# linchaobao/EPPM

Measured on AMD Instinct MI355X. Metric: Mflow-vectors/sec, higher is better.
Workload: dtype f32; 1 GPU; single 1024x436 Sintel-shape synthetic pair per step, full 3-level pyramid, patch_r=9, default defs.h parameters; 1 rank(s), independent pairs; inputs: RGBA planes resident in HBM before the timed region; outputs: interleaved float2 flow left in HBM (the PCIe-inclusive window of the reference API -- host RGB in, host u/v out -- is `host_boundary`, with --full); inputs=device-resident RGBA, outputs=device-resident float2 flow, pairs_in_flight_per_gpu=24, pairs_per_launch=8, contexts_in_flight=3, width=1024, height=436

## Files before the change

### eppm_amd/_lib.py

```python
import ctypes as C
import os

from .build import lib_path


class EppmError(RuntimeError):
    pass


class CParams(C.Structure):
    _fields_ = [("patch_r", C.c_int), ("num_iter", C.c_int), ("search_range", C.c_int), ("num_guess", C.c_int),
                ("seg_len", C.c_int), ("wmf_iters", C.c_int), ("seed", C.c_ulonglong), ("propagation", C.c_int),
                ("levels", C.c_int)]


class CTrackParams(C.Structure):
    _fields_ = [("spacing", C.c_int), ("min_eig", C.c_int64), ("fb_alpha", C.c_float), ("fb_beta", C.c_float), ("mb_alpha", C.c_float),
                ("mb_beta", C.c_float), ("capacity", C.c_int)]


class CTFilterParams(C.Structure):
    _fields_ = [("thresh", C.c_float), ("n_max", C.c_int)]


# ... 64 lines not shown


class CObject(C.Structure):
    _fields_ = [("id", C.c_int32), ("age", C.c_int32), ("area", C.c_int32), ("x0", C.c_int32), ("y0", C.c_int32), ("x1", C.c_int32),
                ("y1", C.c_int32), ("n_flow", C.c_int32), ("sum_x", C.c_int64), ("sum_y", C.c_int64), ("sum_qu", C.c_int64), ("sum_qv", C.c_int64)]

    def as_dict(self):
        return {k: int(getattr(self, k)) for k, _ in self._fields_}


class CObjectsCounts(C.Structure):
    _fields_ = [("n", C.c_int32), ("n_found", C.c_int32), ("n_components", C.c_int32), ("next_id", C.c_int32)]

    def as_dict(self):
        return {k: int(getattr(self, k)) for k, _ in self._fields_}


class CTrackCounts(C.Structure):
    _fields_ = [("live", C.c_int), ("ended", C.c_int), ("seeded", C.c_int), ("dropped", C.c_int), ("frame", C.c_int), ("next_id", C.c_int)]

    def as_dict(self):
        return {k: int(getattr(self, k)) for k, _ in self._fields_}


_lib = None

SYMBOLS = [
    "eppm_default_params", "eppm_create", "eppm_create_batch", "eppm_batch_size", "eppm_batch_set_images", "eppm_batch_set_images_device",
    "eppm_batch_compute", "eppm_batch_compute_device", "eppm_batch_compute_end", "eppm_batch_get_plane", "eppm_destroy", "eppm_set_stream", "eppm_set_images", "eppm_set_images_device",
    "eppm_compute", "eppm_compute_begin", "eppm_compute_end", "eppm_compute_device", "eppm_synchronize", "eppm_num_levels", "eppm_level_dims", "eppm_get_plane",
    "eppm_stage_times", "eppm_clear_stage_times", "eppm_enable_stage_timing", "eppm_last_error", "eppm_version",
    "eppm_device_count", "eppm_set_device", "eppm_malloc_device", "eppm_malloc_pitched", "eppm_free_device",
    "eppm_memcpy_h2d", "eppm_memcpy_d2h", "eppm_memcpy2d_h2d", "eppm_memcpy2d_d2h", "eppm_memset_device",
    "eppm_device_synchronize", "eppm_device_mem_info", "eppm_device_pci_bus_id", "eppm_bind_thread_to_device", "eppm_release_cached_memory", "eppm_set_launcher_stream", "eppm_set_launcher_params", "eppm_launcher_status",
    "baoCudaPatchMatchMultiscalePrepare", "baoCudaCensusTransform", "baoCudaPatchMatch", "baoCudaLeftRightCheck",
    "baoCudaOutlierRemoval", "baoCudaWeightedMedianFilter", "baoCudaFillHole", "baoCudaNNF2Flow", "baoCudaBLF_C2F",
    "baoCudaBLFCostFilterRefine", "baoCudaFlowSmoothing", "eppm_flow_to_color", "eppm_compute_color",
    "eppm_pm_rng_create", "eppm_pm_rng_reset", "eppm_pm_rng_destroy", "eppm_pm_rng_block_states", "eppm_pm_gen_rand_field",
    "eppm_pm_cost_field", "eppm_pm_seg_propagate", "eppm_pm_jump_propagate", "eppm_pm_parallel_propagate", "eppm_pm_random_search", "eppm_gauss_filter_rgba", "eppm_resize_rgba",
    "eppm_resize_flow",
    "eppm_host_register", "eppm_host_unregister", "eppm_host_is_registered", "eppm_host_alloc", "eppm_host_free",
    "eppm_compute_begin_into", "eppm_batch_compute_begin_into",
    "eppm_load_ppm", "eppm_ppm_size", "eppm_save_flo", "eppm_load_flo", "eppm_flo_size", "eppm_flow_error",
    "eppm_flow_error_border", "eppm_flow_error_percentage", "eppm_flow_cutoff", "eppm_flow_to_color_host",
    "eppm_compute_bidirectional", "eppm_compute_bidirectional_device", "eppm_batch_compute_bidirectional", "eppm_set_occlusion_params",
    "eppm_fb_occlusion", "eppm_fb_occlusion_host",
    "eppm_interpolate", "eppm_interpolate_device", "eppm_batch_interpolate", "eppm_interpolate_frames", "eppm_interpolate_host",
    "eppm_track_default_params", "eppm_track_capacity", "eppm_tracker_create", "eppm_tracker_destroy", "eppm_track_step",
    "eppm_track_step_frames", "eppm_tracker_get", "eppm_tracker_get_ended", "eppm_tracker_set", "eppm_track_step_host", "eppm_track_seeds_host",
    "eppm_push_image", "eppm_push_image_device", "eppm_set_temporal", "eppm_temporal_reset", "eppm_temporal_valid", "eppm_temporal_prior_host",
    "eppm_temporal_prior",
    "eppm_batch_set_temporal", "eppm_batch_push_images", "eppm_batch_push_images_device", "eppm_batch_temporal_valid", "eppm_batch_temporal_reset",
    "eppm_temporal_prior_batch",
    "eppm_set_stop_level", "eppm_stop_level", "eppm_flow_upsample",
    "eppm_tfilter_default_params", "eppm_tfilter_create", "eppm_tfilter_create_size", "eppm_tfilter_destroy", "eppm_tfilter_reset", "eppm_tfilter_step",
    "eppm_tfilter_step_frames", "eppm_tfilter_get", "eppm_tfilter_get_device", "eppm_tfilter_get_state", "eppm_tfilter_set_state",
    "eppm_tfilter_seed_host", "eppm_tfilter_step_host",
    "eppm_stab_default_params", "eppm_stab_create", "eppm_stab_create_size", "eppm_stab_destroy", "eppm_stab_reset", "eppm_stab_step",
    "eppm_stab_step_frames", "eppm_stab_get", "eppm_stab_get_device", "eppm_stab_get_mask", "eppm_stab_get_model", "eppm_stab_get_path",
    "eppm_stab_set_path", "eppm_gmotion_fit_host", "eppm_stab_update_host", "eppm_stab_warp_host",
    "eppm_cutdet_default_params", "eppm_cutdet_create", "eppm_cutdet_create_size", "eppm_cutdet_destroy", "eppm_cutdet_step",
    "eppm_cutdet_step_frames", "eppm_cutdet_get", "eppm_cutdet_cuts", "eppm_cutdet_host",
    "eppm_mblur_default_params", "eppm_motion_blur", "eppm_motion_blur_device", "eppm_batch_motion_blur", "eppm_motion_blur_frames",
    "eppm_motion_blur_host",
    "eppm_cmap_default_params", "eppm_cmap_create", "eppm_cmap_create_size", "eppm_cmap_destroy", "eppm_cmap_reset", "eppm_cmap_step",
    "eppm_cmap_step_frames", "eppm_cmap_get_state", "eppm_cmap_set_state", "eppm_cmap_set_layer", "eppm_cmap_render", "eppm_cmap_render_device",
    "eppm_cmap_age", "eppm_cmap_step_host", "eppm_cmap_render_host",
    "eppm_objects_default_params", "eppm_objects_create", "eppm_objects_create_size", "eppm_objects_destroy", "eppm_objects_reset",
    "eppm_objects_step", "eppm_objects_step_frames", "eppm_objects_get", "eppm_objects_get_labels", "eppm_objects_get_state",
    "eppm_objects_set_state", "eppm_objects_label_host", "eppm_objects_carry_host", "eppm_objects_assign_host",
    "eppm_plate_default_params", "eppm_plate_create", "eppm_plate_create_size", "eppm_plate_destroy", "eppm_plate_reset", "eppm_plate_canvas_dims",
    "eppm_plate_step", "eppm_plate_step_frames", "eppm_plate_render", "eppm_plate_render_frames", "eppm_plate_get", "eppm_plate_get_device",
    "eppm_plate_get_mask", "eppm_plate_get_path", "eppm_plate_set_path", "eppm_plate_get_state", "eppm_plate_set_state",
    "eppm_plate_forms_host", "eppm_plate_block_host", "eppm_plate_accumulate_host", "eppm_plate_render_host",
    "eppm_defect_default_params", "eppm_defect_create", "eppm_defect_create_size", "eppm_defect_destroy", "eppm_defect_reset", "eppm_defect_step",
    "eppm_defect_step_frames", "eppm_defect_get", "eppm_defect_get_device", "eppm_defect_get_mask", "eppm_defect_get_stats",
    "eppm_defect_get_state", "eppm_defect_set_state", "eppm_defect_step_host",
    "eppm_deflicker_default_params", "eppm_deflicker_create", "eppm_deflicker_create_size", "eppm_deflicker_destroy", "eppm_deflicker_reset",
    "eppm_deflicker_step", "eppm_deflicker_step_frames", "eppm_deflicker_get", "eppm_deflicker_get_device", "eppm_deflicker_get_field",
    "eppm_deflicker_get_stats", "eppm_deflicker_get_state", "eppm_deflicker_set_state", "eppm_deflicker_step_host",
]


TEST_SYMBOLS = ["eppm_test_set_option", "eppm_test_c2f_refine_batch", "eppm_test_c2f_refine_pre", "eppm_test_c2f_refine_probe", "eppm_probe_c2f_pretest", "eppm_probe_c2f_window", "eppm_probe_dispatch", "eppm_probe_fast_exp", "eppm_probe_div_const", "eppm_probe_delta_table",
                "eppm_probe_unpack_texel", "eppm_probe_pm_parity", "eppm_probe_ctx_rng_states", "eppm_test_pm_search", "eppm_probe_search_pretest", "eppm_probe_launch_log"]

_variant = None


def select_library(variant):
    global _variant
    if _lib is not None and variant != _variant:
        raise EppmError("select_library: a library is loaded already")
    _variant = variant


def lib():
    global _lib
    if _lib is None:
        path = lib_path(_variant)
        if not os.path.exists(path):
            raise EppmError(f"{path} is missing: run eppm_amd.build() (hipcc --offload-arch=gfx950); there is no CPU fallback")
        L = C.CDLL(path)
        L.eppm_last_error.restype = C.c_char_p
        L.eppm_version.restype = C.c_char_p
        _plate_signatures(L)
        _lib = L
    return _lib


def _plate_signatures(L):
    P, I, Z, F = C.c_void_p, C.c_int, C.c_size_t, C.c_float
    sig = {
        "eppm_plate_default_params": [P], "eppm_plate_create": [P, P, P], "eppm_plate_create_size": [I, I, I, I, P, P], "eppm_plate_destroy": [P],
        "eppm_plate_reset": [P, I], "eppm_plate_canvas_dims": [P, P, P], "eppm_plate_step": [P, P, P],
        "eppm_plate_step_frames": [P, I, P, Z, P, P, I], "eppm_plate_render": [P, P, I, P, Z, P],
        "eppm_plate_render_frames": [P, I, P, Z, P, P, P, Z, P], "eppm_plate_get": [P, I, P, Z, P], "eppm_plate_get_device": [P, I, P, Z],
        "eppm_plate_get_mask": [P, I, P], "eppm_plate_get_path": [P, I, P], "eppm_plate_set_path": [P, I, P], "eppm_plate_get_state": [P, I, P],
        "eppm_plate_set_state": [P, I, P], "eppm_plate_forms_host": [P, P, P, P], "eppm_plate_block_host": [P, P, I, I, P],
        "eppm_plate_accumulate_host": [P, P, P, P, I, I, P], "eppm_plate_render_host": [P, P, I, P, P, I, I, P, P, P],
    }
    for name, args in sig.items():
        fn = getattr(L, name, None)
        if fn is None:
            continue
        fn.argtypes = args
        fn.restype = I


def check(status, what=""):
    if status != 0:
        raise EppmError(f"{what}: status {status}: {lib().eppm_last_error().decode()}")


def check_launcher(what=""):
    check(lib().eppm_launcher_status(), what)


LAUNCH_STAGES = ("smoothing", "jbu", "refine", "search", "sweep", "sweeps_merged")


class launch_log:

    def __enter__(self):
        check(lib().eppm_test_set_option(b"launch_log", 1), "launch_log on")
        self._kept = None
        return self

    def entries(self):
        if self._kept is not None:
            return self._kept
        n = lib().eppm_probe_launch_log(None, 0)
        buf = (C.c_int * (6 * max(n, 1)))()
        n = min(n, lib().eppm_probe_launch_log(buf, n))
        return [(LAUNCH_STAGES[buf[6 * i]],) + tuple(buf[6 * i + 1:6 * i + 6]) for i in range(n)]

    def __exit__(self, *exc):
        self._kept = self.entries()
        lib().eppm_test_set_option(b"launch_log", 0)
        return False


def probe_dispatch(stage, *args, nout=1):
    a = (C.c_int * len(args))(*[int(v) for v in args])
    out = (C.c_int * nout)()
    check(lib().eppm_probe_dispatch(stage.encode(), a, len(args), out, nout), f"eppm_probe_dispatch {stage}")
    return tuple(out)
```

### eppm_amd/csrc/api_internal.h

```cpp
#pragma once

#include <ctype.h>
#include <math.h>
#include <sched.h>
#include <stdarg.h>
#include <stdio.h>
#include <stdlib.h>
#include <string.h>

#include <atomic>
#include <chrono>
#include <condition_variable>
#include <map>
#include <mutex>
#include <string>
#include <tuple>
#include <vector>

#include "eppm_internal.h"
#include "host_registry.h"

#define EPPM_HIDDEN __attribute__((visibility("hidden")))

EPPM_HIDDEN int set_err(int code, const char* fmt, ...) __attribute__((format(printf, 2, 3)));
#define HIPCHK(expr)                                                                                         \
    do {                                                                                                     \
        hipError_t e_ = (expr);                                                                              \
        if (e_ != hipSuccess) {                                                                              \
            (void)hipGetLastError();                                                                         \
            return set_err(EPPM_ERR_HIP, "%s failed: %s (%s:%d)", #expr, hipGetErrorString(e_), __FILE__, __LINE__); \
        }                                                                                                    \
    } while (0)
#define CHK(expr)                     \
    do {                              \
        int r_ = (expr);              \
        if (r_ != EPPM_OK) return r_; \
    } while (0)

EPPM_HIDDEN int check_params(const eppm_params& p);
EPPM_HIDDEN void host_pm_lut(int R, std::vector<float>& v);
EPPM_HIDDEN void host_wmf_lut(std::vector<float>& v);
EPPM_HIDDEN void host_blf_lut(std::vector<float>& v);
EPPM_HIDDEN int pyr_init_dim(int* arrH, int* arrW, int h, int w, int maxDepth, double ratio);
EPPM_HIDDEN int upload_lut(float** dst, const std::vector<float>& v);
struct DeltaIndex { int32_t t1[256]; std::vector<float> dval; };
EPPM_HIDDEN const DeltaIndex& delta_index();
EPPM_HIDDEN int upload_lut_delta(float** dst, const std::vector<float>& head, int which);
EPPM_HIDDEN int upload_pm_lut(float** dst, int R);
EPPM_HIDDEN int upload_wmf_lut(float** dst);
EPPM_HIDDEN int upload_blf_lut(float** dst);

#ifdef EPPM_TEST_HOOKS
EPPM_HIDDEN extern std::atomic<int> g_opt_rand_table;
EPPM_HIDDEN extern std::atomic<int> g_opt_sweep_spec;
EPPM_HIDDEN extern std::atomic<int> g_opt_no_split;
EPPM_HIDDEN extern std::atomic<int> g_opt_force_split;
EPPM_HIDDEN extern std::atomic<int> g_opt_search_pre;
static inline int opt_rand_table() { return g_opt_rand_table.load(); }
static inline int opt_sweep_spec() { return g_opt_sweep_spec.load(); }
static inline int opt_no_split() { return g_opt_no_split.load(); }
static inline int opt_force_split() { return g_opt_force_split.load(); }
static inline int opt_search_pre() { return g_opt_search_pre.load(); }
EPPM_HIDDEN extern std::atomic<int> g_opt_c2f_pre;
static inline int opt_c2f_pre() { return g_opt_c2f_pre.load(); }
EPPM_HIDDEN extern std::atomic<int> g_opt_alloc_fill;
static inline int opt_alloc_fill() { return g_opt_alloc_fill.load(); }
EPPM_HIDDEN hipError_t alloc_fill(hipError_t e, void* p, size_t bytes, bool pinned);
#else
static constexpr int opt_rand_table() { return 1; }
static constexpr int opt_sweep_spec() { return -1; }
static constexpr int opt_no_split() { return 0; }
static constexpr int opt_force_split() { return 0; }
static constexpr int opt_search_pre() { return -1; }
static constexpr int opt_c2f_pre() { return -1; }
static constexpr int opt_alloc_fill() { return -1; }
#endif


namespace eppm { struct RngTables; }
struct eppm_pm_rng {
    eppm::RngTables* tables = nullptr;
    const int16_t* rand_tab = nullptr;
    size_t rand_stride = 0;
    int device = 0, w = 0, h = 0, gx = 0, gy = 0, G = 0, per_lane = 0;
    unsigned long long seed = 0;
    uint32_t* init_tab = nullptr;
    uint32_t* iter_tab = nullptr;
    uint32_t* work[2][2] = {{nullptr, nullptr}, {nullptr, nullptr}};
    bool own_work = true;
    int cur[2] = {0, 0};
    uint32_t* skip_mat = nullptr;
    uint32_t skip_weyl = 0;
    eppm::PmRngDev dev() const
    {
        eppm::PmRngDev d;
        d.init_tab = init_tab; d.iter_tab = iter_tab; d.skip_mat = skip_mat;
        d.skip_weyl = skip_weyl; d.per_lane = per_lane; d.gx = gx; d.gy = gy;
        return d;
    }
};
EPPM_HIDDEN int rng_create(eppm_pm_rng** out, int w, int h, const eppm_params& p, bool alloc_work = true);
EPPM_HIDDEN void rng_free(eppm_pm_rng* r);
EPPM_HIDDEN void rngtab_release_idle();

EPPM_HIDDEN hipError_t cache_alloc(void** p, size_t bytes, bool pinned, int device);
EPPM_HIDDEN void cache_free(void* p, size_t bytes, bool pinned, int device);
EPPM_HIDDEN hipError_t pooled_stream_create(hipStream_t* out, int device);
EPPM_HIDDEN void pooled_stream_destroy(hipStream_t s, int device);

EPPM_HIDDEN eppm::PmProblem mk_problem(const eppm::PlanesH& P, float* cost, int16_t* nnf, int16_t* nnf_alt, eppm_pm_rng* rng, int k, float* spec = nullptr,
                                       int32_t* scand = nullptr, uint32_t* wl = nullptr, int16_t* seed = nullptr, float* restw = nullptr);
EPPM_HIDDEN void search(eppm::PmBatch& b, eppm_pm_rng* rng, const float* lut, const eppm_params& prm, hipStream_t s, int launch_no = -1, bool pretest = false);
EPPM_HIDDEN bool sweep_list_on(int mode);
EPPM_DECISION bool sweep_speculative(int iteration, long long pixels, int m);
EPPM_DECISION bool sweeps_merged(int iteration, long long pixels, long long problem_pixels, int m);
EPPM_HIDDEN void sweep(eppm::PmBatch& b, const float* lut, const eppm_params& prm, int dir, hipStream_t s, bool speculative = false);
EPPM_HIDDEN void jump(eppm::PmBatch& b, const float* lut, const eppm_params& prm, hipStream_t s);
EPPM_HIDDEN void neighbor(eppm::PmBatch& b, const float* lut, const eppm_params& prm, int launches, hipStream_t s);
EPPM_HIDDEN void run_patchmatch(eppm::PmBatch& b, eppm_pm_rng* rng, const float* lut, const eppm_params& prm, hipStream_t s, int spec_mode, int pre_from = -1);
EPPM_HIDDEN void pm_start(eppm::PmBatch& b, eppm_pm_rng* rng, const float* lut, const eppm_params& prm, hipStream_t s, int pre_from = -1);
EPPM_HIDDEN void pm_iterate(eppm::PmBatch& b, eppm_pm_rng* rng, const float* lut, const eppm_params& prm, hipStream_t s, int spec_mode, int pre_from = -1);
#ifndef EPPM_SWEEP_CACHE
#define EPPM_SWEEP_CACHE 1
#endif

EPPM_HIDDEN int launcher_finish();

EPPM_HIDDEN int ctx_device(const eppm_ctx* c, int* h, int* w);
EPPM_HIDDEN void ctx_stage_begin(eppm_ctx* c, const char* name);
EPPM_HIDDEN void ctx_stage_end(eppm_ctx* c);

EPPM_HIDDEN int stab_step_on(eppm_stab* f, eppm::StabArgs& in, int slot0, const uint8_t* cut, hipStream_t s, eppm_ctx* timing);
EPPM_HIDDEN const uint8_t* stab_mask_device(const eppm_stab* f, size_t* slot_stride);
EPPM_HIDDEN const char* stab_model_device(const eppm_stab* f, size_t* slot_stride);
```

### eppm_amd/csrc/c2f_device.cuh

```cuda
#pragma once
#include "eppm_device.cuh"

#ifndef EPPM_C2F_UNROLL
#define EPPM_C2F_UNROLL 2
#endif
#ifndef EPPM_C2F_WAVES
#define EPPM_C2F_WAVES 4
#endif
#ifndef EPPM_C2F_WAVES_MIN
#define EPPM_C2F_WAVES_MIN 2
#endif
#define EPPM_C2F_OCC __attribute__((amdgpu_waves_per_eu(EPPM_C2F_WAVES_MIN, EPPM_C2F_WAVES)))
#ifndef EPPM_C2F_WIN_H
#ifdef EPPM_TOL
#define EPPM_C2F_WIN_H 50
#else
#define EPPM_C2F_WIN_H 48
#endif
#endif
#ifndef EPPM_C2F_PASS2
#define EPPM_C2F_PASS2 1
#endif
#ifndef EPPM_C2F_WIN_WAVES
#define EPPM_C2F_WIN_WAVES 4
#endif
#ifndef EPPM_C2F_PRE
#define EPPM_C2F_PRE 1
#endif
#ifndef EPPM_C2F_PRE_ROWS
#define EPPM_C2F_PRE_ROWS 5
#endif
#ifndef EPPM_C2F_PRE_EPS
#define EPPM_C2F_PRE_EPS 0x1p-13f
#endif
#ifndef EPPM_C2F_PRE_PARTS
#define EPPM_C2F_PRE_PARTS 1
#endif
#define EPPM_C2F_PRE_DMIN 0x1p-60f
#define EPPM_C2F_PRE_RHSMIN 0x1p-100f
#ifndef EPPM_C2F_SPLIT_BELOW_WAVES
#define EPPM_C2F_SPLIT_BELOW_WAVES 1024
#endif
#ifndef EPPM_C2F_WINDOW
#define EPPM_C2F_WINDOW 1
#endif
#ifndef EPPM_C2F_WINDOW17
#define EPPM_C2F_WINDOW17 1
#endif
#ifdef EPPM_TOL
#define EPPM_C2F_LOG2 true
#else
#define EPPM_C2F_LOG2 false
#endif
#define EPPM_PRAGMA_(x) _Pragma(#x)
#define EPPM_UNROLL(n) EPPM_PRAGMA_(unroll n)

namespace eppm {

__device__ __forceinline__ Planes to_dev(const PlanesH& h, size_t pstride = 0, unsigned pair = 0)
{
    Planes p;
    p.pk1 = pair_ptr((const float4*)h.pk1, pstride, pair); p.pk2 = pair_ptr((const float4*)h.pk2, pstride, pair);
    p.w = h.w; p.h = h.h; p.pitch = h.pitch;
    return p;
}

__device__ __forceinline__ float4 stage_texel(const uint32_t* __restrict__ pc, const float4* __restrict__ pk, unsigned idx)
{
    if (pc) { const uint32_t w = pc[idx]; return make_texel(w, w >> 24); }
    return pk[idx];
}

__device__ __forceinline__ bool c2f_unknown(float fvx, float fvy) { return fvx > kUnknownFlowThresh || fvy > kUnknownFlowThresh; }
__device__ __forceinline__ int c2f_centre(float f, int x) { return (int)(int16_t)(f2short(f) + x); }
__device__ __forceinline__ void c2f_store_flow(float* flow, int idx, int fx, int fy)
{
    flow[idx * 2] = (float)fx;
    flow[idx * 2 + 1] = (float)fy;
}
__device__ __forceinline__ float c2f_min(float a, float b) { return (a < b) ? a : b; }
__device__ __forceinline__ float c2f_min4(float c1, float c2, float c3, float c4) { return c2f_min(c1, c2f_min(c2, c2f_min(c3, c4))); }
template <class F>
__device__ __forceinline__ void c2f_select_best(float* flow, int x, int y, int ccx, int ccy, int w, int h, F cost_of)
{
    int bx = ccx, by = ccy;
    float min_cost = 999999;
#pragma unroll
    for (int m = 0; m < 3; m++) {
        const int cx = (int)(int16_t)(ccx + m - 1);
        if (cx < 0 || cx >= w) continue;
#pragma unroll
        for (int n = 0; n < 3; n++) {
            const int cy = (int)(int16_t)(ccy + n - 1);
            if (cy < 0 || cy >= h) continue;
            const float cv = cost_of(m, n);
            if (cv < min_cost) { min_cost = cv; bx = cx; by = cy; }
        }
    }
    flow[(y * w + x) * 2] = (float)(bx - x);
    flow[(y * w + x) * 2 + 1] = (float)(by - y);
}

template <int SPLIT>
__device__ __forceinline__ bool c2f_tile_origin(const Planes& P, int& x0, int& y0, int& part)
{
    const int tiles_x = (P.w + kBlock - 1) / kBlock, tiles = tiles_x * ((P.h + kBlock - 1) / kBlock);
    const int per_xcd = (tiles + 7) / 8;
    const int slot = SPLIT ? (blockIdx.x >> 3) / SPLIT : (blockIdx.x >> 3);
    part = SPLIT ? (blockIdx.x >> 3) % SPLIT : -1;
    const int tile = (blockIdx.x & 7) * per_xcd + slot;
    if (slot >= per_xcd || tile >= tiles) return false;
    x0 = (tile % tiles_x) * kBlock; y0 = (tile / tiles_x) * kBlock;
    return true;
}

template <int R> struct C2fSrcTile { static constexpr int TWU = kBlock + 2 * R, TW = (TWU + 15) / 16 * 16; };
template <int R> struct C2fPreList {
    static constexpr int PADB = (C2fSrcTile<R>::TW - C2fSrcTile<R>::TWU) * 16, KROWS = PADB ? (256 * 8 + PADB - 1) / PADB : 0;
    static constexpr int CAP = PADB ? (C2fSrcTile<R>::TWU - KROWS) * (PADB / 2) : 0;
// ... 298 lines not shown
```

### eppm_amd/csrc/context.cpp

```cpp
#include "context.h"

using namespace eppm;

extern "C" int eppm_destroy(eppm_ctx* c)
{
    if (!c) return EPPM_OK;
    (void)hipSetDevice(c->device);
    if (c->stream) (void)hipStreamSynchronize(c->stream);
    c->out_hold.release();
    clear_events(c, c->ev);
    clear_events(c, c->ev_prep);
    for (hipEvent_t e : c->ev_pool) (void)hipEventDestroy(e);
    cache_free(c->slab, c->slab_bytes, false, c->device);
    if (c->h_color) (void)hipHostFree(c->h_color);
    for (int q = 0; q < 2; q++) {
        cache_free(c->h_rgb[q], c->h_rgb_bytes, true, c->device);
        if (c->ev_rgb[q]) (void)hipEventDestroy(c->ev_rgb[q]);
    }
    if (c->ev_h2d) (void)hipEventDestroy(c->ev_h2d);
    cache_free(c->h_flow, c->h_flow_bytes, true, c->device);
    cache_free(c->bwd, c->bwd_bytes, false, c->device);
    cache_free(c->h_bwd, c->h_bwd_bytes, true, c->device);
    cache_free(c->itp, c->itp_bytes, false, c->device);
    cache_free(c->h_itp, c->h_itp_bytes, true, c->device);
// ... 11 lines not shown
    struct Entry { int device, R; float *pm, *wmf, *blf; };
    static std::mutex mu;
    static std::vector<Entry> tab;
    std::lock_guard<std::mutex> lk(mu);
    for (const Entry& e : tab)
        if (e.device == device && e.R == R) { *pm = e.pm; *wmf = e.wmf; *blf = e.blf; return EPPM_OK; }
    Entry e{device, R, nullptr, nullptr, nullptr};
    CHK(upload_pm_lut(&e.pm, R));
    CHK(upload_wmf_lut(&e.wmf));
    CHK(upload_blf_lut(&e.blf));
    tab.push_back(e);
    *pm = e.pm; *wmf = e.wmf; *blf = e.blf;
    return EPPM_OK;
}

static int ctx_alloc(eppm_ctx* c)
{
    const int h = c->h, w = c->w;
    Carve cv;
    auto pitch_of = [](size_t row_bytes) { return (row_bytes + 255) & ~(size_t)255; };
    c->raw_pitch = pitch_of((size_t)w * 4);
    for (uint32_t** p : {&c->raw1, &c->raw2}) cv.plane(p, c->raw_pitch * h);
    for (int i = 0; i < c->nl; i++) {
        c->ipitch[i] = pitch_of((size_t)c->W[i] * 4);
        c->cpitch[i] = pitch_of((size_t)c->W[i]);
        const size_t n = (size_t)c->W[i] * c->H[i];
        for (uint32_t** p : {&c->img1[i], &c->img2[i], &c->tmpu[i]}) cv.plane(p, c->ipitch[i] * c->H[i]);
        for (void** p : {&c->pk1[i], &c->pk2[i]}) cv.plane(p, n * 16);
        for (uint32_t** p : {&c->pc1[i], &c->pc2[i]}) cv.plane(p, n * 4);
        for (uint8_t** p : {&c->cen1[i], &c->cen2[i]}) cv.plane(p, c->cpitch[i] * c->H[i]);
        for (float** p : {&c->flow[i], &c->flow_tmp[i]}) cv.plane(p, n * 8);
        if (i < c->nl - 1 && c2f_refine_wants_split(c->W[i], c->H[i], c->prm.patch_r, 1, c->opt_no_split != 0)) cv.plane(&c->c2f_cost9[i], n * 36 * 4);
    }
    const int L = c->nl - 1;
    const size_t n2 = (size_t)c->W[L] * c->H[L];
#ifndef EPPM_TOL
    if (c->prm.patch_r == 9)
#endif
    {
        c->pp_pad = (c->prm.patch_r + 2) & ~1;
        c->pp_pitch = parity_pitch(c->W[L], c->pp_pad);
        for (uint32_t** p : {&c->pp1, &c->pp2}) cv.plane(p, (size_t)2 * c->H[L] * c->pp_pitch * 4);
    }
    for (int16_t** p : {&c->nnf1, &c->nnf2, &c->nnf_tmp, &c->nnf_tmp2}) cv.plane(p, n2 * 4);
    for (float** p : {&c->cost1, &c->cost2}) cv.plane(p, n2 * 4);
    for (float** p : {&c->spec1, &c->spec2}) cv.plane(p, n2 * 4 * 4);
    if (pm_search_pretest_form(c->W[L], c->H[L], c->prm.patch_r, 2, c->npairs))
        for (float** p : {&c->restw1, &c->restw2}) cv.plane(p, n2 * 4);
    for (int32_t** p : {&c->scand1, &c->scand2}) cv.plane(p, n2 * 4 * 4);
    for (uint32_t** p : {&c->wl1, &c->wl2}) cv.plane(p, pm_worklist_words(c->W[L], c->H[L], c->prm.seg_len) * 4);
    for (int16_t** p : {&c->seed1, &c->seed2}) cv.plane(p, n2 * 4 * 4);
    cv.plane(&c->wmf_ws, wmf_workspace_words(c->W[L], c->H[L], c->prm.wmf_iters) * 4);
    cv.plane(&c->d_rgb, (size_t)h * w * 3 * 2);
    cv.plane(&c->d_color, (size_t)h * w * 4);
    cv.plane(&c->d_uv, (size_t)h * w * 8);
    CHK(rng_create(&c->rng, c->W[L], c->H[L], c->prm, false));
    const size_t rng_bytes = (size_t)c->rng->gx * c->rng->gy * 64 * 6 * 4;
    for (int k = 0; k < 2; k++)
        for (int q = 0; q < 2; q++) cv.plane(&c->rng->work[k][q], rng_bytes);
    c->stride = (cv.off + 4095) & ~(size_t)4095;
    CHK(cv.alloc(&c->slab, &c->slab_bytes, c->stride * c->npairs, c->device, (std::to_string(c->npairs) + " slab(s)").c_str()));
    CHK(shared_luts(c->device, c->prm.patch_r, &c->lut_pm, &c->lut_wmf, &c->lut_blf));
    c->out_u.assign(c->npairs, nullptr);
    c->out_v.assign(c->npairs, nullptr);
    for (auto* v : {&c->tmp_snap, &c->tmp_valid, &c->tmp_seeded, &c->tmp_cut}) v->assign(c->npairs, 0);
    return EPPM_OK;
}

extern "C" int eppm_create_batch(eppm_ctx** out, int h, int w, int device, const eppm_params* params, int npairs)
{
    if (!out) return set_err(EPPM_ERR_ARG, "eppm_create: NULL out");
    *out = nullptr;
    if (npairs < 1 || npairs > 4096) return set_err(EPPM_ERR_ARG, "eppm_create_batch: npairs %d out of range [1,4096]", npairs);
    if (h < 4 || w < 4 || h > 32767 || w > 32767) return set_err(EPPM_ERR_ARG, "eppm_create: size %dx%d out of range (NNF coordinates are int16)", w, h);
    if ((unsigned long long)h * (unsigned long long)w * 16ULL >= (1ULL << 32))
        return set_err(EPPM_ERR_ARG, "eppm_create: size %dx%d out of range (texel planes are addressed with 32-bit byte offsets)", w, h);
    eppm_params p;
    eppm_default_params(&p);
    if (params) p = *params;
    CHK(check_params(p));
    HIPCHK(hipSetDevice(device));
    eppm_ctx* c = new eppm_ctx();
    c->device = device; c->prm = p; c->h = h; c->w = w; c->npairs = npairs; c->n_active = 1;
    c->opt_sweep_spec = opt_sweep_spec(); c->opt_no_split = opt_no_split(); c->opt_search_pre = opt_search_pre(); c->opt_c2f_pre = opt_c2f_pre();
    c->nl = pyr_init_dim(c->H, c->W, h, w, p.levels, 0.5f);
    const int L = c->nl - 1;
    if (c->H[L] < 1 || c->W[L] < 1 || (c->W[L] + p.seg_len - 1) / p.seg_len > 1024 || (c->H[L] + p.seg_len - 1) / p.seg_len > 1024) {
        delete c;
        return set_err(EPPM_ERR_ARG, "eppm_create: unsupported size %dx%d", w, h);
    }
    const hipError_t e = pooled_stream_create(&c->stream, c->device);
    if (e != hipSuccess) { delete c; return set_err(EPPM_ERR_HIP, "hipStreamCreate: %s", hipGetErrorString(e)); }
    c->own_stream = true;
    int r = ctx_alloc(c);
    if (r != EPPM_OK) { eppm_destroy(c); return r; }
    *out = c;
    return EPPM_OK;
}

extern "C" int eppm_create(eppm_ctx** out, int h, int w, int device, const eppm_params* params)
{
    return eppm_create_batch(out, h, w, device, params, 1);
}

extern "C" int eppm_batch_size(const eppm_ctx* c) { return c ? c->npairs : 0; }

extern "C" int eppm_set_stream(eppm_ctx* c, void* s)
{
    if (!c) return set_err(EPPM_ERR_ARG, "NULL ctx");
    if (c->own_stream && c->stream) { (void)hipStreamSynchronize(c->stream); pooled_stream_destroy(c->stream, c->device); }
    c->stream = (hipStream_t)s;
    c->own_stream = false;
    return EPPM_OK;
}

extern "C" int eppm_num_levels(const eppm_ctx* c) { return c ? c->nl : 0; }
extern "C" int eppm_level_dims(const eppm_ctx* c, int level, int* h, int* w)
{
    if (!c || level < 0 || level >= c->nl) return set_err(EPPM_ERR_ARG, "bad level");
    if (h) *h = c->H[level];
    if (w) *w = c->W[level];
    return EPPM_OK;
}
extern "C" int eppm_enable_stage_timing(eppm_ctx* c, int on)
{
    if (!c) return set_err(EPPM_ERR_ARG, "NULL ctx");
    c->timing = (on == 2) ? 2 : (on != 0);
    return EPPM_OK;
}

int ctx_device(const eppm_ctx* c, int* h, int* w)
{
    *h = c->h;
    *w = c->w;
    return c->device;
}

void ctx_stage_begin(eppm_ctx* c, const char* name) { stage_begin(c, c->ev, name); }
void ctx_stage_end(eppm_ctx* c) { stage_end(c, c->ev); }

extern "C" int eppm_synchronize(eppm_ctx* c)
{
    if (!c) return set_err(EPPM_ERR_ARG, "NULL ctx");
    HIPCHK(hipStreamSynchronize(c->stream));
    return EPPM_OK;
}

extern "C" int eppm_stage_times(eppm_ctx* c, const char** names, float* ms, int max)
{
    if (!c) return 0;
    (void)hipStreamSynchronize(c->stream);
    int n = 0;
    for (auto* v : {&c->ev_prep, &c->ev})
        for (auto& e : *v) {
            if (n >= max) return n;
            float t = 0;
            if (hipEventElapsedTime(&t, e.a, e.b) != hipSuccess) t = -1;
            names[n] = e.name; ms[n] = t; n++;
        }
    return n;
}

extern "C" int eppm_clear_stage_times(eppm_ctx* c)
{
    if (!c) return set_err(EPPM_ERR_ARG, "NULL ctx");
    (void)hipStreamSynchronize(c->stream);
    clear_events(c, c->ev);
// ... 86 lines not shown
```

### eppm_amd/csrc/context.h

```cpp
#pragma once

#include <algorithm>

#include "api_internal.h"

struct StageEv { const char* name; hipEvent_t a, b; };

struct eppm_ctx {
    int device = 0;
    hipStream_t stream = nullptr;
    bool own_stream = false;
    int opt_sweep_spec = -1, opt_no_split = 0, opt_search_pre = -1, opt_c2f_pre = -1;
    eppm_params prm;
    int h = 0, w = 0, nl = 0;
    int stop_level = 0;
    int npairs = 1, n_active = 1;
    char* slab = nullptr;
    size_t stride = 0;
    int H[eppm::kMaxLevels], W[eppm::kMaxLevels];
    size_t ipitch[eppm::kMaxLevels], cpitch[eppm::kMaxLevels];
    uint32_t *raw1 = nullptr, *raw2 = nullptr;
    size_t raw_pitch = 0;
    uint32_t *img1[eppm::kMaxLevels] = {}, *img2[eppm::kMaxLevels] = {}, *tmpu[eppm::kMaxLevels] = {};
    uint8_t *cen1[eppm::kMaxLevels] = {}, *cen2[eppm::kMaxLevels] = {};
    void *pk1[eppm::kMaxLevels] = {}, *pk2[eppm::kMaxLevels] = {};
    uint32_t *pc1[eppm::kMaxLevels] = {}, *pc2[eppm::kMaxLevels] = {};
    uint32_t *pp1 = nullptr, *pp2 = nullptr;
    int pp_pitch = 0, pp_pad = 0;
    int16_t *nnf1 = nullptr, *nnf2 = nullptr, *nnf_tmp = nullptr, *nnf_tmp2 = nullptr;
    float *cost1 = nullptr, *cost2 = nullptr;
    float *spec1 = nullptr, *spec2 = nullptr;
    int32_t *scand1 = nullptr, *scand2 = nullptr;
    uint32_t *wl1 = nullptr, *wl2 = nullptr;
    float *restw1 = nullptr, *restw2 = nullptr;
    int16_t *seed1 = nullptr, *seed2 = nullptr;
    uint32_t* wmf_ws = nullptr;
    bool flow_pending = false;
    float *flow[eppm::kMaxLevels] = {}, *flow_tmp[eppm::kMaxLevels] = {};
    float* c2f_cost9[eppm::kMaxLevels] = {};
    float *lut_pm = nullptr, *lut_wmf = nullptr, *lut_blf = nullptr;
    eppm_pm_rng* rng = nullptr;
    float* d_uv = nullptr;
    uint32_t* d_color = nullptr;
    uint32_t* h_color = nullptr;
    uint8_t* d_rgb = nullptr;
    size_t slab_bytes = 0, h_rgb_bytes = 0, h_flow_bytes = 0;
    uint8_t* h_rgb[2] = {nullptr, nullptr};
    hipEvent_t ev_rgb[2] = {nullptr, nullptr};
    hipEvent_t ev_h2d = nullptr;
    int rgb_cur = 0;
    float* h_flow = nullptr;
    std::vector<float*> out_u, out_v;
    eppm::HostHold out_hold;
    bool have_images = false, have_flow = false;
    char* bwd = nullptr;
    size_t bwd_stride = 0, bwd_bytes = 0, h_bwd_bytes = 0;
    float* bflow[eppm::kMaxLevels] = {};
    float* d_buv = nullptr;
    uint8_t *occ1 = nullptr, *occ2 = nullptr;
    uint8_t* h_bwd = nullptr;
    float occ_alpha = 0.01f, occ_beta = 0.5f;
    bool have_bwd = false;
    bool bwd_images = false;
    char* itp = nullptr;
    size_t itp_bytes = 0, itp_plane = 0, h_itp_bytes = 0;
    uint64_t* itp_keys = nullptr;
    int32_t *itp_fill1 = nullptr, *itp_fill2 = nullptr;
    uint8_t* itp_rgb = nullptr;
    uint8_t* h_itp = nullptr;
    char* mbl = nullptr;
    size_t mbl_bytes = 0, mbl_plane = 0, mbl_tplane = 0, h_mbl_bytes = 0;
    uint32_t* mbl_packed = nullptr;
    uint64_t* mbl_tkeys = nullptr;
    uint8_t* mbl_rgb = nullptr;
    uint8_t* h_mbl = nullptr;
    bool temporal = false;
    std::vector<uint8_t> tmp_snap;
    std::vector<uint8_t> tmp_valid;
    std::vector<uint8_t> tmp_seeded;
    std::vector<uint8_t> tmp_cut;
    char* tmp = nullptr;
    size_t tmp_bytes = 0, tmp_stride = 0;
    int16_t *prev_fwd = nullptr, *prev_bwd = nullptr, *prior1 = nullptr, *prior2 = nullptr, *nnf_init1 = nullptr, *nnf_init2 = nullptr;
    float *cost_init1 = nullptr, *cost_init2 = nullptr;
    int32_t* tmp_keys = nullptr;
    void tmp_drop() { std::fill(tmp_valid.begin(), tmp_valid.end(), 0); std::fill(tmp_snap.begin(), tmp_snap.end(), 0); std::fill(tmp_cut.begin(), tmp_cut.end(), 0); }
    int timing = 0;
    std::vector<StageEv> ev;
    std::vector<StageEv> ev_prep;
    std::vector<hipEvent_t> ev_pool;
    eppm::Batch bt() const { return eppm::Batch{n_active, stride}; }
    template <class T> T* of_pair(T* p, int k) const { return (T*)((char*)p + (size_t)k * stride); }
    template <class T> T* of_bwd_pair(T* p, int k) const { return (T*)((char*)p + (size_t)k * bwd_stride); }
};

static inline eppm::PlanesH planes(const eppm_ctx* c, int l, bool swap)
{
    eppm::PlanesH p;
    p.pk1 = swap ? c->pk2[l] : c->pk1[l];
    p.pk2 = swap ? c->pk1[l] : c->pk2[l];
    p.w = c->W[l]; p.h = c->H[l];
    p.pitch = c->W[l];
    p.pc1 = swap ? c->pc2[l] : c->pc1[l];
    p.pc2 = swap ? c->pc1[l] : c->pc2[l];
    if (l == c->nl - 1 && c->pp1) {
        p.pp1 = swap ? c->pp2 : c->pp1;
        p.pp2 = swap ? c->pp1 : c->pp2;
        p.pp_pitch = c->pp_pitch; p.pp_pad = c->pp_pad;
    }
    return p;
}

static inline hipEvent_t pool_event(eppm_ctx* c)
{
    hipEvent_t e = nullptr;
    if (!c->ev_pool.empty()) { e = c->ev_pool.back(); c->ev_pool.pop_back(); }
    else (void)hipEventCreate(&e);
    return e;
}
static inline bool stage_on(const eppm_ctx* c, bool dominant) { return c->timing == 1 || (c->timing == 2 && dominant); }
static inline void stage_begin(eppm_ctx* c, std::vector<StageEv>& v, const char* name, bool dominant = false)
{
    if (!stage_on(c, dominant)) return;
    StageEv e;
    e.name = name;
    e.a = pool_event(c);
    e.b = pool_event(c);
    (void)hipEventRecord(e.a, c->stream);
    v.push_back(e);
}
static inline void stage_end(eppm_ctx* c, std::vector<StageEv>& v, bool dominant = false)
{
    if (!stage_on(c, dominant)) return;
    (void)hipEventRecord(v.back().b, c->stream);
// ... 44 lines not shown
```

### eppm_amd/csrc/ctx_compute.cpp

```cpp
#include "context.h"
#include "temporal.h"

using namespace eppm;

static int tmp_alloc(eppm_ctx* c)
{
    if (c->tmp) return EPPM_OK;
    const int L = c->nl - 1;
    const size_t n2 = (size_t)c->W[L] * c->H[L];
    Carve cv;
    for (int16_t** p : {&c->prev_fwd, &c->prev_bwd, &c->prior1, &c->prior2, &c->nnf_init1, &c->nnf_init2}) cv.plane(p, n2 * 4);
    for (float** p : {&c->cost_init1, &c->cost_init2}) cv.plane(p, n2 * 4);
    cv.plane(&c->tmp_keys, n2 * 4 * 2);
    c->tmp_stride = cv.off;
    CHK(cv.alloc(&c->tmp, &c->tmp_bytes, c->tmp_stride * c->npairs, c->device, "temporal planes"));
    for (int k = 0; k < c->npairs; k++) launch_temporal_keys_init((int32_t*)((char*)c->tmp_keys + (size_t)k * c->tmp_stride), (int)(2 * n2), c->stream);
    HIPCHK(hipGetLastError());
    return EPPM_OK;
}

static int set_temporal(eppm_ctx* c, int on)
{
    c->temporal = on != 0;
    if (!on) c->tmp_drop();
    return EPPM_OK;
}
extern "C" int eppm_set_temporal(eppm_ctx* c, int on)
{
    if (!c) return set_err(EPPM_ERR_ARG, "eppm_set_temporal: NULL ctx");
    if (on && c->npairs != 1) return set_err(EPPM_ERR_ARG, "eppm_set_temporal: a batch context streams through eppm_batch_set_temporal (one clip per slot)");
    return set_temporal(c, on);
}
extern "C" int eppm_temporal_reset(eppm_ctx* c)
{
    if (!c) return set_err(EPPM_ERR_ARG, "eppm_temporal_reset: NULL ctx");
    return eppm_batch_temporal_reset(c, 0);
}
extern "C" int eppm_temporal_valid(const eppm_ctx* c) { return eppm_batch_temporal_valid(c, 0); }

extern "C" int eppm_batch_set_temporal(eppm_ctx* c, int on)
{
    if (!c) return set_err(EPPM_ERR_ARG, "eppm_batch_set_temporal: NULL ctx");
    return set_temporal(c, on);
}
extern "C" int eppm_batch_temporal_reset(eppm_ctx* c, int pair)
{
    if (!c) return set_err(EPPM_ERR_ARG, "eppm_batch_temporal_reset: NULL ctx");
    if (pair >= c->npairs) return set_err(EPPM_ERR_ARG, "eppm_batch_temporal_reset: pair %d, context holds %d", pair, c->npairs);
    for (int k = pair < 0 ? 0 : pair; k < (pair < 0 ? c->npairs : pair + 1); k++) c->tmp_valid[k] = c->tmp_snap[k] = 0;
    return EPPM_OK;
}
extern "C" int eppm_batch_temporal_valid(const eppm_ctx* c, int pair)
{
    return c && pair >= 0 && pair < c->npairs && c->temporal && c->tmp_valid[pair] ? 1 : 0;
}

struct Branch {
    int16_t *&nnf, *&nnf_alt;
    float* cost;
    uint32_t* const* guide;
    bool swap, bwd, dominant;
    int16_t* snapshot;
    float *a[kMaxLevels], *b[kMaxLevels];
};

enum { kStageUp, kStageRefine, kStageBlf, kStageJbu };
static const struct EPPM_HIDDEN LevelStageNames {
    char s[4][2][kMaxLevels][24];
    LevelStageNames()
    {
        const char* base[4] = {"upsample", "c2f_refine", "flow_blf", "flow_jbu"};
        for (int k = 0; k < 4; k++)
            for (int b = 0; b < 2; b++)
                for (int l = 0; l < kMaxLevels; l++) snprintf(s[k][b][l], sizeof s[k][b][l], "%s%s_L%d", base[k], b ? "_bwd" : "", l);
    }
} level_stage;

static void branch_nnf2flow(eppm_ctx* c, Branch& d)
{
    hipStream_t s = c->stream;
    const Batch bt = c->bt();
    const int L = c->nl - 1, lw = c->W[L], lh = c->H[L], gp = (int)(c->ipitch[L] / 4);
    launch_outlier(d.nnf_alt, d.cost, d.nnf, lw, lh, lw, lw, s, bt);
    std::swap(d.nnf, d.nnf_alt);
    if (launch_wmf(d.nnf, d.nnf_alt, d.guide[L], gp, lw, lh, lw, c->lut_wmf, c->prm.wmf_iters, 1, c->wmf_ws, s, bt) != d.nnf)
        std::swap(d.nnf, d.nnf_alt);
    launch_fill_holes(d.nnf_alt, d.nnf, d.guide[L], gp, lw, lh, lw, s, bt);
    std::swap(d.nnf, d.nnf_alt);
    if (d.snapshot) launch_nnf2flow_snapshot(d.a[L], lw, d.snapshot, c->tmp_stride, d.nnf, lw, lw, lh, s, bt);
    else launch_nnf2flow(d.a[L], lw, d.nnf, lw, lw, lh, s, bt);
}

static int branch_c2f(eppm_ctx* c, Branch& d, int (*keep)(eppm_ctx*, int, float*))
{
    hipStream_t s = c->stream;
    const Batch bt = c->bt();
    const int L = c->nl - 1;
    auto blf = [&](float* dst, const float* src, int l) { launch_flow_blf(dst, src, d.guide[l], (int)(c->ipitch[l] / 4), c->W[l], c->H[l], c->W[l], c->lut_blf, s, bt); };
    const int stop = c->stop_level;
    float* r = d.a[L];
    for (int l = L - 1; l >= 0; l--) {
        if (l < stop) {
            stage_begin(c, c->ev, level_stage.s[kStageJbu][d.bwd][l]);
            float* out = (r == d.b[l]) ? d.a[l] : d.b[l];
            launch_flow_jbu(out, r, d.guide[l], (int)(c->ipitch[l] / 4), c->W[l], c->H[l], c->W[l + 1], c->H[l + 1], c->lut_blf, s, bt);
            r = out;
            CHK(keep(c, l, r));
            stage_end(c, c->ev);
            continue;
        }
        stage_begin(c, c->ev, level_stage.s[kStageUp][d.bwd][l]);
        launch_resize_flow(d.a[l], c->H[l], c->W[l], r, c->H[l + 1], c->W[l + 1], 2.0f, 2.0f, s, bt);
        stage_end(c, c->ev);
        stage_begin(c, c->ev, level_stage.s[kStageRefine][d.bwd][l], d.dominant);
        launch_c2f_refine(planes(c, l, d.swap), d.a[l], c->lut_pm, c->prm.patch_r, c->c2f_cost9[l], s, bt, c->opt_no_split != 0, c->opt_c2f_pre);
        stage_end(c, c->ev, d.dominant);
        stage_begin(c, c->ev, level_stage.s[kStageBlf][d.bwd][l]);
        blf(d.b[l], d.a[l], l);
        r = d.b[l];
        if (l > 0) CHK(keep(c, l, r));
        stage_end(c, c->ev);
    }
    if (stop > 0) return EPPM_OK;
    stage_begin(c, c->ev, d.bwd ? "flow_blf_bwd_final" : "flow_blf_final");
    float* out = (r == d.b[0]) ? d.a[0] : d.b[0];
    blf(out, r, 0);
    CHK(keep(c, 0, out));
    stage_end(c, c->ev);
    return EPPM_OK;
}

static int keep_fwd(eppm_ctx* c, int l, float* r)
{
    if (r != c->flow[l]) std::swap(c->flow[l], c->flow_tmp[l]);
    return EPPM_OK;
}

static int compute_all(eppm_ctx* c)
{
    if (!c->have_images) return set_err(EPPM_ERR_STATE, "eppm_compute: no images set");
    HIPCHK(hipSetDevice(c->device));
    c->have_bwd = false;
    hipStream_t s = c->stream;
    const Batch bt = c->bt();
    const int L = c->nl - 1, lw = c->W[L], lh = c->H[L];

    const bool tmode = c->temporal;
    bool seeded = false;
    std::fill(c->tmp_seeded.begin(), c->tmp_seeded.end(), 0);
    if (tmode) {
        CHK(tmp_alloc(c));
        TemporalArgs a{};
        for (int k = 0; k < bt.n; k++)
            if (c->tmp_valid[k]) { a.armed[k >> 5] |= 1u << (k & 31); seeded = true; }
        if (seeded) {
            a.prev[0] = c->prev_fwd; a.prior[0] = c->prior1; a.keys[0] = c->tmp_keys; a.step[0] = 1;
            a.prev[1] = c->prev_bwd; a.prior[1] = c->prior2; a.keys[1] = c->tmp_keys + (size_t)lw * lh; a.step[1] = -1;
            a.w = lw; a.h = lh; a.ndir = 2; a.nslots = bt.n; a.stride = c->tmp_stride;
            stage_begin(c, c->ev, "temporal_advect");
            launch_temporal_splat(a, s);
            launch_temporal_gather(a, s);
            stage_end(c, c->ev);
        }
    }
    std::fill(c->tmp_snap.begin(), c->tmp_snap.end(), 0);

    const size_t pm_entry = c->ev.size();
    stage_begin(c, c->ev, "patchmatch");
    {
        PmBatch b;
        b.n = 2; b.cpitch = lw; b.npitch = lw; b.npairs = bt.n; b.stride = bt.stride;
        b.cache_plane = (size_t)lw * lh;
        b.seed_plane = (size_t)lw * lh * 2;
        b.wl_units = pm_worklist_units(lw, lh, c->prm.seg_len);
        b.p[0] = mk_problem(planes(c, L, false), c->cost1, c->nnf1, c->nnf_tmp, c->rng, 0, c->spec1, EPPM_SWEEP_CACHE ? c->scand1 : nullptr, sweep_list_on(c->opt_sweep_spec) ? c->wl1 : nullptr, c->seed1, c->restw1);
        b.p[1] = mk_problem(planes(c, L, true), c->cost2, c->nnf2, c->nnf_tmp2, c->rng, 1, c->spec2, EPPM_SWEEP_CACHE ? c->scand2 : nullptr, sweep_list_on(c->opt_sweep_spec) ? c->wl2 : nullptr, c->seed2, c->restw2);
        if (!seeded) run_patchmatch(b, c->rng, c->lut_pm, c->prm, s, c->opt_sweep_spec, c->opt_search_pre);
        else {
            pm_start(b, c->rng, c->lut_pm, c->prm, s, c->opt_search_pre);
            PmSeed sd;
            sd.prior[0] = c->prior1; sd.nnf_init[0] = c->nnf_init1; sd.cost_init[0] = c->cost_init1;
            sd.prior[1] = c->prior2; sd.nnf_init[1] = c->nnf_init2; sd.cost_init[1] = c->cost_init2;
            sd.stride = c->tmp_stride;
            stage_begin(c, c->ev, "temporal_select");
            launch_pm_cost_select(b, sd, c->lut_pm, c->prm.patch_r, s);
            stage_end(c, c->ev);
            pm_iterate(b, c->rng, c->lut_pm, c->prm, s, c->opt_sweep_spec, c->opt_search_pre);
        }
    }
    stage_end_at(c, c->ev, pm_entry);
    if (tmode) launch_temporal_snapshot(c->prev_bwd, c->tmp_stride, c->nnf2, lw, lw, lh, s, bt);

    stage_begin(c, c->ev, "l2_post");
    launch_lr_check(c->nnf1, c->cost1, c->nnf2, lw, lh, lw, lw, s, bt);
    launch_lr_check(c->nnf2, c->cost2, c->nnf1, lw, lh, lw, lw, s, bt);
    Branch d{c->nnf1, c->nnf_tmp, c->cost1, c->img1, false, false, true, tmode ? c->prev_fwd : nullptr};
    for (int l = 0; l <= L; l++) { d.a[l] = c->flow[l]; d.b[l] = c->flow_tmp[l]; }
    branch_nnf2flow(c, d);
    stage_end(c, c->ev);
    CHK(branch_c2f(c, d, keep_fwd));
    HIPCHK(hipGetLastError());
    c->have_flow = true;
    for (int k = 0; k < bt.n; k++) {
        c->tmp_snap[k] = tmode && !c->tmp_cut[k];
        c->tmp_seeded[k] = tmode && c->tmp_valid[k];
    }
    std::fill(c->tmp_valid.begin(), c->tmp_valid.end(), 0);
    return EPPM_OK;
}


static int bwd_alloc(eppm_ctx* c)
{
    if (c->bwd) return EPPM_OK;
    Carve cv;
    for (int l = 0; l < c->nl; l++) cv.plane(&c->bflow[l], (size_t)c->W[l] * c->H[l] * 8);
    const size_t n = (size_t)c->h * c->w;
    cv.plane(&c->d_buv, n * 10);
    c->bwd_stride = (cv.off + 4095) & ~(size_t)4095;
    CHK(cv.alloc(&c->bwd, &c->bwd_bytes, c->bwd_stride * c->npairs, c->device, "backward planes"));
    c->occ1 = (uint8_t*)c->d_buv + n * 8;
    c->occ2 = c->occ1 + n;
    return EPPM_OK;
}

static int keep_bwd(eppm_ctx* c, int l, float* src)
{
    const size_t bytes = (size_t)c->W[l] * c->H[l] * 8;
    for (int k = 0; k < c->n_active; k++)
        HIPCHK(hipMemcpyAsync(c->of_bwd_pair(c->bflow[l], k), c->of_pair(src, k), bytes, hipMemcpyDeviceToDevice, c->stream));
    return EPPM_OK;
}

static int backward_all(eppm_ctx* c)
{
    const int L = c->nl - 1;
    Branch d{c->nnf2, c->nnf_tmp2, c->cost2, c->img2, true, true, false, nullptr};
    for (int l = 0; l <= L; l++) { d.a[l] = c->flow_tmp[l]; d.b[l] = c->d_uv; }
    stage_begin(c, c->ev, "l2_post_bwd");
    branch_nnf2flow(c, d);
    if (L > 0) CHK(keep_bwd(c, L, d.a[L]));
    stage_end(c, c->ev);
    CHK(branch_c2f(c, d, keep_bwd));

    stage_begin(c, c->ev, "fb_occlusion");
    launch_fb_occlusion(c->occ1, c->occ2, c->flow[0], c->stride, c->bflow[0], c->bwd_stride, c->h, c->w, c->occ_alpha, c->occ_beta, c->n_active, 2, c->stream);
    stage_end(c, c->ev);
    HIPCHK(hipGetLastError());
    c->have_bwd = true;
    c->bwd_images = true;
    return EPPM_OK;
}

static int compute_bidir_all(eppm_ctx* c)
{
    if (!c->have_images) return set_err(EPPM_ERR_STATE, "eppm_compute_bidirectional: no images set");
    HIPCHK(hipSetDevice(c->device));
    CHK(bwd_alloc(c));
    CHK(compute_all(c));
    return backward_all(c);
}

extern "C" int eppm_compute_device(eppm_ctx* c, void* d_flow)
{
    if (!c) return set_err(EPPM_ERR_ARG, "NULL ctx");
    CHK(compute_all(c));
    if (d_flow) HIPCHK(hipMemcpyAsync(d_flow, c->flow[0], (size_t)c->h * c->w * 8, hipMemcpyDeviceToDevice, c->stream));
    return EPPM_OK;
}

extern "C" int eppm_batch_compute_device(eppm_ctx* c, void* const* d_flows)
{
    if (!c) return set_err(EPPM_ERR_ARG, "NULL ctx");
    CHK(compute_all(c));
    if (d_flows)
        for (int k = 0; k < c->n_active; k++)
            if (d_flows[k]) HIPCHK(hipMemcpyAsync(d_flows[k], c->of_pair(c->flow[0], k), (size_t)c->h * c->w * 8, hipMemcpyDeviceToDevice, c->stream));
    return EPPM_OK;
}

static int compute_begin_impl(eppm_ctx* c, int n_out, float* const* u, float* const* v, bool bidir)
{
    CHK(bidir ? compute_bidir_all(c) : compute_all(c));
    const size_t n = (size_t)c->h * c->w;
    launch_split_flow(c->d_uv, c->flow[0], (int)n, c->stream, c->bt());
    if (bidir) {
        launch_split_flow(c->d_buv, c->bflow[0], (int)n, c->stream, Batch{c->n_active, c->bwd_stride});
        HIPCHK(pinned_lazy(&c->h_bwd, &c->h_bwd_bytes, n * 10 * c->npairs, c->device));
        for (int k = 0; k < c->n_active; k++)
            HIPCHK(hipMemcpyAsync(c->h_bwd + (size_t)k * n * 10, c->of_bwd_pair(c->d_buv, k), n * 10, hipMemcpyDeviceToHost, c->stream));
    }
    for (int k = 0; k < c->n_active; k++) {
        float* du = (u && k < n_out) ? u[k] : nullptr;
        float* dv = (v && k < n_out) ? v[k] : nullptr;
        const float* src = c->of_pair(c->d_uv, k);
        if (du && dv && c->out_hold.add2(du, dv, n * 4)) {
            HIPCHK(hipMemcpyAsync(du, src, n * 4, hipMemcpyDeviceToHost, c->stream));
            HIPCHK(hipMemcpyAsync(dv, src + n, n * 4, hipMemcpyDeviceToHost, c->stream));
            c->out_u[k] = du; c->out_v[k] = dv;
            continue;
        }
        HIPCHK(pinned_lazy(&c->h_flow, &c->h_flow_bytes, n * 8 * c->npairs, c->device));
        HIPCHK(hipMemcpyAsync(c->h_flow + (size_t)k * n * 2, src, n * 8, hipMemcpyDeviceToHost, c->stream));
        c->out_u[k] = c->out_v[k] = nullptr;
    }
    c->flow_pending = true;
    return EPPM_OK;
}
static int compute_begin(eppm_ctx* c, int n_out, float* const* u, float* const* v, bool bidir = false)
{
    const int r = compute_begin_impl(c, n_out, u, v, bidir);
    if (r != EPPM_OK && !c->out_hold.v.empty()) {
        (void)hipStreamSynchronize(c->stream);
        c->out_hold.release();
    }
    return r;
}

extern "C" int eppm_compute_begin(eppm_ctx* c)
{
    if (!c) return set_err(EPPM_ERR_ARG, "eppm_compute_begin: NULL ctx");
    return compute_begin(c, 0, nullptr, nullptr);
}

extern "C" int eppm_compute_begin_into(eppm_ctx* c, float* u, float* v)
{
    if (!c || !u || !v) return set_err(EPPM_ERR_ARG, "eppm_compute_begin_into: NULL argument");
    return compute_begin(c, 1, &u, &v);
}

extern "C" int eppm_batch_compute_begin_into(eppm_ctx* c, float* const* u, float* const* v)
{
    if (!c || !u || !v) return set_err(EPPM_ERR_ARG, "eppm_batch_compute_begin_into: NULL argument");
    return compute_begin(c, c->n_active, u, v);
}

static int compute_end(eppm_ctx* c, int n_out, float* const* u, float* const* v)
{
    if (!c->flow_pending) return set_err(EPPM_ERR_STATE, "eppm_compute_end without eppm_compute_begin");
    HIPCHK(hipSetDevice(c->device));
    const hipError_t es = hipStreamSynchronize(c->stream);
    c->out_hold.release();
    HIPCHK(es);
    c->flow_pending = false;
    const size_t n = (size_t)c->h * c->w;
    for (int k = 0; k < n_out && k < c->n_active; k++) {
        if (!u[k] || !v[k]) continue;
        const float* fu = c->out_u[k] ? c->out_u[k] : c->h_flow + (size_t)k * n * 2;
        const float* fv = c->out_v[k] ? c->out_v[k] : c->h_flow + (size_t)k * n * 2 + n;
        if (u[k] != fu) memcpy(u[k], fu, n * sizeof(float));
        if (v[k] != fv) memcpy(v[k], fv, n * sizeof(float));
    }
    return EPPM_OK;
}

extern "C" int eppm_compute_end(eppm_ctx* c, float* u, float* v)
{
    if (!c || !u || !v) return set_err(EPPM_ERR_ARG, "eppm_compute_end: NULL argument");
    return compute_end(c, 1, &u, &v);
}

// ... 88 lines not shown
```

### eppm_amd/csrc/ctx_images.cpp

```cpp
#include "context.h"

using namespace eppm;

static int prepare(eppm_ctx* c, bool only2 = false)
{
    stage_begin(c, c->ev_prep, "prepare");
    hipStream_t s = c->stream;
    const Batch bt = c->bt();
    uint32_t **p1 = c->img1, **p2 = c->img2, **tmp = c->tmpu;
    const int p0 = (int)(c->ipitch[0] / 4);
    if (only2) launch_gauss_rgba(p2[0], c->raw2, p0, c->H[0], c->W[0], .5f, 2, s, bt);
    else launch_gauss_rgba2(p1[0], c->raw1, p2[0], c->raw2, p0, c->H[0], c->W[0], .5f, 2, s, bt);
    const float ratio = 0.5f;
    const float baseSigma = (1 / ratio - 1);
    const int n = (int)(log(0.25) / (double)logf(ratio));
    const float nSigma = baseSigma * n;
    for (int i = 1; i < c->nl; i++) {
        const int j = (i <= n) ? 0 : i - n;
        const float sigma = (i <= n) ? baseSigma * i : nSigma;
        const float r = (i <= n) ? (float)pow(ratio, i) : (float)pow(ratio, i) * c->W[0] / c->W[j];
        const int radius = (int)(sigma * 3);
        const int pj = (int)(c->ipitch[j] / 4), pi = (int)(c->ipitch[i] / 4);
        if (gauss_decimate2_ok(c->H[i], c->W[i], c->H[j], c->W[j], r, radius)) {
            if (only2) launch_gauss_decimate2(p2[i], p2[j], p2[i], p2[j], 1, pi, c->H[i], c->W[i], pj, c->H[j], c->W[j], sigma, radius, s, bt);
            else launch_gauss_decimate2(p1[i], p1[j], p2[i], p2[j], 2, pi, c->H[i], c->W[i], pj, c->H[j], c->W[j], sigma, radius, s, bt);
        } else {
            for (int k = only2 ? 1 : 0; k < 2; k++) {
                uint32_t** pyr = k ? p2 : p1;
                launch_gauss_rgba(tmp[j], pyr[j], pj, c->H[j], c->W[j], sigma, radius, s, bt);
                launch_resize_rgba(pyr[i], pi, c->H[i], c->W[i], tmp[j], pj, c->H[j], c->W[j], r, s, bt);
            }
        }
    }
    CensusBatch cb;
    cb.n = 0;
    for (int k = only2 ? 1 : 0; k < 2; k++)
        for (int i = 0; i < c->nl; i++) {
            CensusJob& J = cb.job[cb.n++];
            J.census = k ? c->cen2[i] : c->cen1[i]; J.cpitch = (int)c->cpitch[i];
            J.texels = k ? c->pk2[i] : c->pk1[i];   J.tpitch = c->W[i];
            J.img = k ? c->img2[i] : c->img1[i];    J.ipitch = (int)(c->ipitch[i] / 4);
            J.w = c->W[i]; J.h = c->H[i]; J.first_block = 0;
            J.packed = k ? c->pc2[i] : c->pc1[i];
        }
    launch_census_batch(cb, s, bt);
    if (c->pp1) {
        const int L = c->nl - 1;
        if (!only2) launch_parity_planes(c->pp1, c->pp_pitch, c->pp_pad, c->pc1[L], c->W[L], c->W[L], c->H[L], s, bt);
        launch_parity_planes(c->pp2, c->pp_pitch, c->pp_pad, c->pc2[L], c->W[L], c->W[L], c->H[L], s, bt);
    }
    stage_end(c, c->ev_prep);
    HIPCHK(hipGetLastError());
    c->have_images = true;
    c->have_flow = false;
    c->bwd_images = false;
    return EPPM_OK;
}

static int upload_rgb(eppm_ctx* c, uint8_t* dst, const uint8_t* src, size_t row_stride, HostHold& hold, int slot, bool* direct, bool* staged)
{
    const size_t row = (size_t)c->w * 3, img = row * c->h, span = row_stride * (c->h - 1) + row;
    if (hold.add(src, span)) {
        if (row_stride == row) HIPCHK(hipMemcpyAsync(dst, src, img, hipMemcpyHostToDevice, c->stream));
        else HIPCHK(hipMemcpy2DAsync(dst, row, src, row_stride, row, c->h, hipMemcpyHostToDevice, c->stream));
        *direct = true;
        return EPPM_OK;
    }
    const int q = c->rgb_cur;
    if (!*staged) {
        HIPCHK(pinned_lazy(&c->h_rgb[q], &c->h_rgb_bytes, img * 2 * c->npairs, c->device));
        if (!c->ev_rgb[q]) HIPCHK(hipEventCreateWithFlags(&c->ev_rgb[q], hipEventDisableTiming));
        else HIPCHK(hipEventSynchronize(c->ev_rgb[q]));
    }
    uint8_t* h = c->h_rgb[q] + (size_t)slot * img;
    copy_rows(h, row, src, row_stride, row, c->h);
    HIPCHK(hipMemcpyAsync(dst, h, img, hipMemcpyHostToDevice, c->stream));
    *staged = true;
    return EPPM_OK;
}
static int upload_done(eppm_ctx* c, bool direct, bool staged)
{
    if (staged) {
        HIPCHK(hipEventRecord(c->ev_rgb[c->rgb_cur], c->stream));
        c->rgb_cur ^= 1;
    }
    if (direct) {
        if (!c->ev_h2d) HIPCHK(hipEventCreateWithFlags(&c->ev_h2d, hipEventDisableTiming));
        HIPCHK(hipEventRecord(c->ev_h2d, c->stream));
    }
    return EPPM_OK;
}

static int set_images_host_impl(eppm_ctx* c, int n, const uint8_t* const* rgb1, const uint8_t* const* rgb2, size_t row_stride, HostHold& hold)
{
    if (row_stride < (size_t)c->w * 3) return set_err(EPPM_ERR_ARG, "eppm_set_images: row_stride %zu < 3*w", row_stride);
    HIPCHK(hipSetDevice(c->device));
    const size_t img = (size_t)c->w * 3 * c->h;
    for (int k = 0; k < n; k++)
        if (!rgb1[k] || !rgb2[k]) return set_err(EPPM_ERR_ARG, "eppm_set_images: NULL image");
    bool staged = false, direct = false;
    for (int k = 0; k < n; k++)
        for (int f = 0; f < 2; f++)
            CHK(upload_rgb(c, c->of_pair(c->d_rgb, k) + (size_t)f * img, f ? rgb2[k] : rgb1[k], row_stride, hold, k * 2 + f, &direct, &staged));
    CHK(upload_done(c, direct, staged));
    c->n_active = n;
    c->tmp_drop();
    const int p0 = (int)(c->raw_pitch / 4);
    launch_rgb_to_rgba(c->raw1, p0, c->d_rgb, c->h, c->w, c->stream, c->bt());
    launch_rgb_to_rgba(c->raw2, p0, c->d_rgb + img, c->h, c->w, c->stream, c->bt());
    const int r = prepare(c);
    if (direct) HIPCHK(hipEventSynchronize(c->ev_h2d));
    return r;
}
static int set_images_host(eppm_ctx* c, int n, const uint8_t* const* rgb1, const uint8_t* const* rgb2, size_t row_stride)
{
    HostHold hold;
    const int r = set_images_host_impl(c, n, rgb1, rgb2, row_stride, hold);
    if (r != EPPM_OK && !hold.v.empty()) (void)hipStreamSynchronize(c->stream);
    return r;
}

extern "C" int eppm_set_images(eppm_ctx* c, const uint8_t* rgb1, const uint8_t* rgb2, size_t row_stride)
{
    if (!c || !rgb1 || !rgb2) return set_err(EPPM_ERR_ARG, "eppm_set_images: NULL argument");
    return set_images_host(c, 1, &rgb1, &rgb2, row_stride);
}

extern "C" int eppm_batch_set_images(eppm_ctx* c, int n, const uint8_t* const* rgb1, const uint8_t* const* rgb2, size_t row_stride)
{
    if (!c || !rgb1 || !rgb2) return set_err(EPPM_ERR_ARG, "eppm_batch_set_images: NULL argument");
    if (n < 1 || n > c->npairs) return set_err(EPPM_ERR_ARG, "eppm_batch_set_images: %d pairs, context holds %d", n, c->npairs);
    return set_images_host(c, n, rgb1, rgb2, row_stride);
}

static int set_images_device(eppm_ctx* c, int n, const void* const* d1, const void* const* d2, size_t pitch)
{
    if (pitch < (size_t)c->w * 4 || (pitch & 3)) return set_err(EPPM_ERR_ARG, "eppm_set_images_device: bad pitch %zu", pitch);
    HIPCHK(hipSetDevice(c->device));
    for (int k = 0; k < n; k++) {
        if (!d1[k] || !d2[k]) return set_err(EPPM_ERR_ARG, "eppm_set_images_device: NULL image");
        HIPCHK(hipMemcpy2DAsync(c->of_pair(c->raw1, k), c->raw_pitch, d1[k], pitch, (size_t)c->w * 4, c->h, hipMemcpyDeviceToDevice, c->stream));
        HIPCHK(hipMemcpy2DAsync(c->of_pair(c->raw2, k), c->raw_pitch, d2[k], pitch, (size_t)c->w * 4, c->h, hipMemcpyDeviceToDevice, c->stream));
    }
    c->n_active = n;
    c->tmp_drop();
    return prepare(c);
}

extern "C" int eppm_set_images_device(eppm_ctx* c, const void* d1, const void* d2, size_t pitch)
{
    if (!c || !d1 || !d2) return set_err(EPPM_ERR_ARG, "eppm_set_images_device: NULL argument");
    return set_images_device(c, 1, &d1, &d2, pitch);
}

extern "C" int eppm_batch_set_images_device(eppm_ctx* c, int n, const void* const* d_rgba1, const void* const* d_rgba2, size_t pitch)
{
    if (!c || !d_rgba1 || !d_rgba2) return set_err(EPPM_ERR_ARG, "eppm_batch_set_images_device: NULL argument");
    if (n < 1 || n > c->npairs) return set_err(EPPM_ERR_ARG, "eppm_batch_set_images_device: %d pairs, context holds %d", n, c->npairs);
    return set_images_device(c, n, d_rgba1, d_rgba2, pitch);
}

static int push_check(eppm_ctx* c, const char* what, bool batch = false)
{
    if (!batch && c->npairs != 1) return set_err(EPPM_ERR_ARG, "%s: a batch context takes one frame per slot (eppm_batch_push_images)", what);
    if (!c->have_images) return set_err(EPPM_ERR_STATE, "%s: no pair set yet (eppm_set_images first)", what);
    if (c->flow_pending) return set_err(EPPM_ERR_STATE, "%s: an eppm_compute_begin is pending", what);
    return EPPM_OK;
}
static void push_swap(eppm_ctx* c, const uint8_t* new_clip = nullptr)
{
    for (int k = 0; k < c->n_active; k++) {
        const bool cut = new_clip && new_clip[k];
        c->tmp_valid[k] = c->temporal && c->tmp_snap[k] && !cut;
        c->tmp_snap[k] = 0;
        c->tmp_cut[k] = cut;
    }
    std::swap(c->raw1, c->raw2);
    for (int l = 0; l < c->nl; l++) {
        std::swap(c->img1[l], c->img2[l]);
        std::swap(c->cen1[l], c->cen2[l]);
        std::swap(c->pk1[l], c->pk2[l]);
        std::swap(c->pc1[l], c->pc2[l]);
    }
    std::swap(c->pp1, c->pp2);
}

static int push_image_host_impl(eppm_ctx* c, const uint8_t* rgb, size_t row_stride, HostHold& hold)
{
    if (row_stride < (size_t)c->w * 3) return set_err(EPPM_ERR_ARG, "eppm_push_image: row_stride %zu < 3*w", row_stride);
    HIPCHK(hipSetDevice(c->device));
    uint8_t* dst = c->d_rgb + (size_t)c->w * 3 * c->h;
    bool staged = false, direct = false;
    CHK(upload_rgb(c, dst, rgb, row_stride, hold, 1, &direct, &staged));
    CHK(upload_done(c, direct, staged));
    push_swap(c);
    launch_rgb_to_rgba(c->raw2, (int)(c->raw_pitch / 4), dst, c->h, c->w, c->stream, c->bt());
    const int r = prepare(c, true);
    if (direct) HIPCHK(hipEventSynchronize(c->ev_h2d));
    return r;
}

extern "C" int eppm_push_image(eppm_ctx* c, const uint8_t* rgb, size_t row_stride)
{
    if (!c || !rgb) return set_err(EPPM_ERR_ARG, "eppm_push_image: NULL argument");
    CHK(push_check(c, "eppm_push_image"));
    HostHold hold;
    const int r = push_image_host_impl(c, rgb, row_stride, hold);
    if (r != EPPM_OK && !hold.v.empty()) (void)hipStreamSynchronize(c->stream);
    return r;
}

extern "C" int eppm_push_image_device(eppm_ctx* c, const void* d_rgba, size_t pitch)
{
    if (!c || !d_rgba) return set_err(EPPM_ERR_ARG, "eppm_push_image_device: NULL argument");
    CHK(push_check(c, "eppm_push_image_device"));
    if (pitch < (size_t)c->w * 4 || (pitch & 3)) return set_err(EPPM_ERR_ARG, "eppm_push_image_device: bad pitch %zu", pitch);
    HIPCHK(hipSetDevice(c->device));
    HIPCHK(hipMemcpy2DAsync(c->raw1, c->raw_pitch, d_rgba, pitch, (size_t)c->w * 4, c->h, hipMemcpyDeviceToDevice, c->stream));
    push_swap(c);
    return prepare(c, true);
}

static int push_images_host_impl(eppm_ctx* c, int n, const uint8_t* const* rgb, size_t row_stride, const uint8_t* new_clip, HostHold& hold)
{
    if (row_stride < (size_t)c->w * 3) return set_err(EPPM_ERR_ARG, "eppm_batch_push_images: row_stride %zu < 3*w", row_stride);
    for (int k = 0; k < n; k++)
        if (!rgb[k]) return set_err(EPPM_ERR_ARG, "eppm_batch_push_images: NULL image");
    HIPCHK(hipSetDevice(c->device));
    const size_t img = (size_t)c->w * 3 * c->h;
// ... 36 lines not shown
```

### eppm_amd/csrc/eppm_internal.h

```cpp
#pragma once

#include <hip/hip_runtime.h>
#include <stddef.h>
#include <stdint.h>

#include <atomic>

#include "../../include/eppm.h"

namespace eppm {

constexpr int kMaxLevels = 8;
constexpr int kNumLevels = 3;
constexpr int kBlock = 16;
constexpr int kMaxS = 32;
constexpr int kWmfRadius = 4;
constexpr int kBlfRadius = 10;
constexpr int kDeltaSlots = 800;

struct Batch {
    int n;
    size_t stride;
};
constexpr Batch kOnePair = {1, 0};

#define EPPM_DECISION __attribute__((visibility("hidden")))
enum LaunchStage { kLaunchSmoothing = 0, kLaunchJbu, kLaunchRefine, kLaunchSearch, kLaunchSweep, kLaunchSweepsMerged };
typedef void (*LaunchNoteFn)(int stage, int w, int h, int npairs, int form, int extra);
extern EPPM_DECISION std::atomic<LaunchNoteFn> g_launch_note;
inline void launch_note(int stage, int w, int h, int npairs, int form, int extra = 0)
{
    if (LaunchNoteFn f = g_launch_note.load(std::memory_order_relaxed)) f(stage, w, h, npairs, form, extra);
}

struct PlanesH {
    const void* pk1;
    const void* pk2;
    int w, h, pitch;
    const uint32_t* pc1 = nullptr;
    const uint32_t* pc2 = nullptr;
    const uint32_t* pp1 = nullptr;
    const uint32_t* pp2 = nullptr;
    int pp_pitch = 0, pp_pad = 0;
};
inline int parity_pitch(int w, int pad) { return (w + 2 * pad + 1) / 2 + 1; }
void launch_parity_planes(uint32_t* pp, int pp_pitch, int pad, const uint32_t* pc, int pc_pitch, int w, int h, hipStream_t s, Batch bt = kOnePair);

void launch_gauss_rgba(uint32_t* out, const uint32_t* in, int pitch_px, int h, int w, float sigma, int radius, hipStream_t s, Batch bt = kOnePair);
bool gauss_decimate2_ok(int outH, int outW, int h, int w, float ratio, int radius);
void launch_gauss_decimate2(uint32_t* out0, const uint32_t* in0, uint32_t* out1, const uint32_t* in1, int nimg, int out_pitch_px, int outH,
                            int outW, int pitch_px, int h, int w, float sigma, int radius, hipStream_t s, Batch bt = kOnePair);
void launch_gauss_rgba2(uint32_t* out0, const uint32_t* in0, uint32_t* out1, const uint32_t* in1, int pitch_px, int h, int w, float sigma,
                        int radius, hipStream_t s, Batch bt = kOnePair);
struct CensusJob { uint8_t* census; int cpitch; void* texels; int tpitch; const uint32_t* img; int ipitch; int w, h; int first_block;
                   uint32_t* packed = nullptr; };
struct CensusBatch { int n; CensusJob job[2 * kMaxLevels]; };
void launch_census_batch(CensusBatch& B, hipStream_t s, Batch bt = kOnePair);
void launch_resize_rgba(uint32_t* out, int out_pitch_px, int outH, int outW, const uint32_t* in, int in_pitch_px, int h, int w,
                        float ratio, hipStream_t s, Batch bt = kOnePair);
void launch_census(uint8_t* census, int cpitch, void* texels, int tpitch, const uint32_t* img, int ipitch, int w, int h, hipStream_t s);
void launch_pack(void* texels, int tpitch, const uint32_t* img, int ipitch, const uint8_t* census, int cpitch, int w, int h, hipStream_t s);
void launch_delta_values(float* t2, int n, int which, hipStream_t s);
void launch_rgb_to_rgba(uint32_t* out, int pitch_px, const uint8_t* rgb, int h, int w, hipStream_t s, Batch bt = kOnePair);

struct PmProblem {
    PlanesH P;
    float* cost;
    int16_t* nnf;
    int16_t* nnf_alt;
    float* spec = nullptr;
    int32_t* scand = nullptr;
    uint32_t* wl = nullptr;
    int16_t* seed = nullptr;
    uint32_t* rng_work;
    uint32_t* rng_work_next;
    float* restw = nullptr;
};
struct PmBatch {
    PmProblem p[2];
    int n;
    int cpitch, npitch;
    int npairs = 1;
    size_t stride = 0;
    size_t cache_plane = 0;
    int wl_units = 0;
    int sweep_seq = 0;
    size_t seed_plane = 0;
    int merged_it = 0;
    int seg_len = 0, nseg_row = 0, nseg_col = 0;
};
int pm_worklist_units(int w, int h, int seg_len);
inline size_t pm_worklist_words(int w, int h, int seg_len) { return 16 + 10 * (size_t)pm_worklist_units(w, h, seg_len); }
struct PmRngDev {
    const uint32_t* init_tab;
    const uint32_t* iter_tab;
    const uint32_t* skip_mat;
    uint32_t skip_weyl;
    int per_lane;
    int gx, gy;
    const int16_t* rand_tab = nullptr;
};
void launch_pm_rand_table(const PmRngDev& rng, uint32_t* work, int16_t* tab, int G, hipStream_t s);
void launch_pm_init_field(const PmBatch& b, const PmRngDev& rng, hipStream_t s);
void launch_pm_cost_field(const PmBatch& b, const float* lut, int R, hipStream_t s);
int pm_parity_kernels(int R);
bool launch_pm_sweep(PmBatch& b, const float* lut, int R, int seg_len, int dir, hipStream_t s, bool speculative = false);
bool launch_pm_sweeps_merged(PmBatch& b, const float* lut, int R, int seg_len, int iteration, hipStream_t s);
void launch_pm_jump(const PmBatch& b, const float* lut, int R, int step, hipStream_t s);
void launch_pm_neighbor(const PmBatch& b, const float* lut, int R, hipStream_t s);
void launch_pm_random_search(const PmBatch& b, const PmRngDev& rng, const float* lut, int R, int search_range, int num_guess,
                             hipStream_t s, bool pretest = false);
void launch_pm_rest_weight(const PmBatch& b, const float* lut, int R, hipStream_t s);
bool pm_search_pretest_ready(const PmBatch& b, const PmRngDev& rng, int R);
struct PmPretestSums { float* n[2]; float* d[2]; };
void launch_pm_pretest_probe(const PmBatch& b, const float* lut, int R, const PmPretestSums& out, hipStream_t s);
EPPM_DECISION bool pm_search_pretest_form(int w, int h, int R, int problems, int npairs);
EPPM_DECISION bool pm_search_pretest(int iteration, int w, int h, int R, int problems, int npairs);
EPPM_DECISION void pm_search_pretest_knobs(int R, int* row0, int* rows, int* from, float* eps);
EPPM_DECISION int pm_search_rows(int w, int h, int R, int problems, int npairs, bool table);
struct SweepForm { int lpc; bool small, pre, tile; };
EPPM_DECISION SweepForm pm_sweep_form(int w, int h, int R, int seg_len, int dir, int problems, int npairs);

struct PmSeed {
    const int16_t* prior[2];
    int16_t* nnf_init[2];
    float* cost_init[2];
    size_t stride = 0;
};
void launch_pm_cost_select(const PmBatch& b, const PmSeed& seed, const float* lut, int R, hipStream_t s);

constexpr int kTemporalMaxSlots = 4096;
struct TemporalArgs {
    const int16_t* prev[2];
    int16_t* prior[2];
    int32_t* keys[2];
    int step[2];
    int w, h, ndir;
    int nslots;
    size_t stride;
    uint32_t armed[kTemporalMaxSlots / 32];
};
void launch_temporal_keys_init(int32_t* keys, int n, hipStream_t s);
void launch_temporal_splat(const TemporalArgs& a, hipStream_t s);
void launch_temporal_gather(const TemporalArgs& a, hipStream_t s);
void launch_temporal_snapshot(int16_t* prev, size_t prev_stride, const int16_t* nnf, int nnf_pitch, int w, int h, hipStream_t s, Batch bt = kOnePair);
void launch_nnf2flow_snapshot(float* flow, int flow_pitch, int16_t* prev, size_t prev_stride, const int16_t* nnf, int nnf_pitch, int w, int h,
                              hipStream_t s, Batch bt = kOnePair);

void launch_lr_check(int16_t* nnf1, float* cost1, const int16_t* nnf2, int w, int h, int cost_pitch, int nnf_pitch, hipStream_t s, Batch bt = kOnePair);
void launch_outlier(int16_t* nnf_out, float* cost, const int16_t* nnf_in, int w, int h, int cost_pitch, int nnf_pitch, hipStream_t s, Batch bt = kOnePair);
size_t wmf_workspace_words(int w, int h, int num_iter);
int16_t* launch_wmf(int16_t* buf_a, int16_t* buf_b, const uint32_t* img, int ipitch, int w, int h, int nnf_pitch,
                    const float* wmf_lut, int num_iter, int only_occlusion, uint32_t* ws, hipStream_t s, Batch bt = kOnePair);
void launch_fill_holes(int16_t* nnf_out, const int16_t* nnf_in, const uint32_t* img, int ipitch, int w, int h, int nnf_pitch,
                       hipStream_t s, Batch bt = kOnePair);
void launch_nnf2flow(float* flow, int flow_pitch, const int16_t* nnf, int nnf_pitch, int w, int h, hipStream_t s, Batch bt = kOnePair);

void launch_resize_flow(float* out, int outH, int outW, const float* in, int h, int w, float ratio, float post_scale, hipStream_t s, Batch bt = kOnePair);
void launch_mul_scalar(float* flow, float scale, int h, int w, hipStream_t s);
EPPM_DECISION int c2f_refine_split_factor(int w, int h, int R, int npairs = 1, bool no_split = false);
bool c2f_refine_wants_split(int w, int h, int R, int npairs = 1, bool no_split = false);
bool c2f_window_span(int R, int* span_x, int* span_y);
void launch_c2f_refine(const PlanesH& P, float* flow, const float* lut, int R, float* cost9, hipStream_t s, Batch bt = kOnePair, bool no_split = false,
                       int pre = -1, unsigned* stat = nullptr, float* probe = nullptr);
void c2f_pretest_knobs(int R, int* on, int* row0, int* rows, int* cap, int* parts, float* eps, float* dmin, float* rhsmin);
void launch_flow_blf(float* out, const float* in, const uint32_t* img, int ipitch, int w, int h, int flow_pitch,
                     const float* blf_lut, hipStream_t s, Batch bt = kOnePair);
EPPM_DECISION int flow_blf_pixels_per_lane(int w, int h, int npairs = 1);
void launch_flow_jbu(float* out, const float* in_coarse, const uint32_t* img, int ipitch, int w, int h, int wc, int hc, const float* blf_lut,
                     hipStream_t s, Batch bt = kOnePair);

void launch_split_flow(float* uv, const float* flow, int n, hipStream_t s, Batch bt = kOnePair);

void launch_fb_occlusion(uint8_t* occ1, uint8_t* occ2, const float* fwd, size_t fwd_stride, const float* bwd, size_t bwd_stride, int h, int w,
                         float alpha, float beta, int npairs, int ndir, hipStream_t s);

constexpr int kInterpChunk = 4;
struct InterpArgs {
    const uint8_t* img1;
    const uint8_t* img2;
    size_t img_pitch, img_stride;
    const float* flow;
    size_t flow_stride;
    const uint8_t* occ1;
    const uint8_t* occ2;
    size_t occ_stride;
    uint64_t* keys;
    int32_t* fill1;
    int32_t* fill2;
    size_t plane;
    uint8_t* rgb;
    uint8_t* rgba[kInterpChunk];
    size_t rgba_pitch;
    int h, w, nt;
    float t[kInterpChunk];
};
void launch_interp_splat(const InterpArgs& a, int npairs, hipStream_t s);
void launch_interp_fill(const InterpArgs& a, int npairs, hipStream_t s);
void launch_interp_blend(const InterpArgs& a, int npairs, hipStream_t s);

struct MBlurArgs {
    const uint8_t* img;
    size_t img_pitch, img_stride;
    const float* flow;
    size_t flow_stride;
    uint32_t* packed;
    uint64_t* tkeys;
    size_t plane, tplane;
    uint8_t* rgb;
    uint8_t* rgba;
    size_t rgba_pitch;
    int h, w, tiles_x, tiles_y;
    float shutter, max_radius;
    int taps;
};
void launch_mblur_pack(const MBlurArgs& a, int npairs, hipStream_t s);
void launch_mblur_gather(const MBlurArgs& a, int npairs, hipStream_t s);

enum {
    kTrackCntLive, kTrackCntNextId, kTrackCntFrame, kTrackCntDropped, kTrackCntEnded, kTrackCntSeeded,
    kTrackCntIdBase, kTrackCntSurv, kTrackCntPrevLive, kTrackCntSeeded0, kTrackCntDropped0, kTrackCntN = 16
};
struct TrackRec;
struct TrackDev {
    struct {
        int spacing;
        long long min_eig;
        float fb_alpha, fb_beta, mb_alpha, mb_beta;
    } p;
    int cap, ncells, ncx;
    float* npos;
    uint8_t* stat;
    TrackRec* ended;
    int32_t* ended_reason;
    uint8_t* cov;
    uint8_t* flags;
    int32_t *blk_s, *blk_e;
    int32_t* blk_c;
    int32_t* cnt;
};
struct TrackIn {
    const uint8_t* img1;
    const uint8_t* img2;
    size_t pitch;
    const float* fwd;
    const float* bwd;
    int h, w;
};
void launch_track_seed0(const TrackDev& d, const TrackIn& in, TrackRec* cur, hipStream_t s);
void launch_track_advance(const TrackDev& d, const TrackIn& in, const TrackRec* cur, hipStream_t s);
// ... 193 lines not shown
```

### eppm_amd/csrc/k_c2f_refine.hip

```cpp
#include <type_traits>

#include "c2f_device.cuh"
#include "eppm_internal.h"

namespace eppm {

__constant__ C2fTables<9> c2f_tab9 = make_c2f_tables<9>();
__constant__ C2fTables<17> c2f_tab17 = make_c2f_tables<17>();
template <> __device__ __forceinline__ const C2fTables<9>& c2f_tables<9>() { return c2f_tab9; }
template <> __device__ __forceinline__ const C2fTables<17>& c2f_tables<17>() { return c2f_tab17; }

__global__ __launch_bounds__(256) void k_c2f_refine(PlanesH Ph, float* __restrict__ flow_, const float* __restrict__ lut, int R, size_t pstride)
{
    __shared__ EPPM_LUT_ALIGN PatchLut L;
    load_patch_lut(L, lut, R, threadIdx.y * kBlock + threadIdx.x, 256);
    __syncthreads();
    const Planes P = to_dev(Ph, pstride, blockIdx.z);
    float* __restrict__ flow = pair_ptr(flow_, pstride, blockIdx.z);
    const int x = blockIdx.x * kBlock + threadIdx.x, y = blockIdx.y * kBlock + threadIdx.y;
    if (x >= P.w || y >= P.h) return;
    const float fvx = flow[(y * P.w + x) * 2], fvy = flow[(y * P.w + x) * 2 + 1];
    if (c2f_unknown(fvx, fvy)) { c2f_store_flow(flow, y * P.w + x, 0, 0); return; }
    const int ccx = c2f_centre(fvx, x), ccy = c2f_centre(fvy, y);
    int bx = ccx, by = ccy;
// ... 6 lines not shown
            const int cy = (int)(int16_t)(ccy + n - 1);
            if (cx < 0 || cy < 0 || cx >= P.w || cy >= P.h) continue;
            const float cv = patch_dist_planefit(P, L, R, x, y, cx, cy);
            if (cv < min_cost) { min_cost = cv; bx = cx; by = cy; }
        }
    }
    flow[(y * P.w + x) * 2] = (float)(bx - x);
    flow[(y * P.w + x) * 2 + 1] = (float)(by - y);
}

template <int R, int SPLIT>
__global__ __launch_bounds__(256) EPPM_C2F_OCC void k_c2f_refine_tiled(PlanesH Ph, float* __restrict__ flow_, const float* __restrict__ lut,
                                                                       float* __restrict__ cost9_, size_t pstride)
{
    float* __restrict__ flow = pair_ptr(flow_, pstride, blockIdx.y);
    float* __restrict__ cost9 = pair_ptr_opt(cost9_, pstride, blockIdx.y);
    constexpr int TWU = C2fSrcTile<R>::TWU, TW = C2fSrcTile<R>::TW;
    __shared__ EPPM_LUT_ALIGN PatchLutT<R + 1> L;
    __shared__ float4 s_src[TWU * TW];
    const int tid = threadIdx.y * kBlock + threadIdx.x;
    load_patch_lut<EPPM_C2F_LOG2>(L, lut, R, tid, 256);
    const Planes P = to_dev(Ph, pstride, blockIdx.y);
    int x0, y0, part;
    if (!c2f_tile_origin<SPLIT>(P, x0, y0, part)) return;
    const int m_only = (SPLIT == 3) ? part : -1;
    for (int t = tid; t < TWU * TWU; t += 256) {
        const int ry = t / TWU, rx = t % TWU;
        const int sy = iclamp(y0 + ry - R, 0, P.h - 1), sx = iclamp(x0 + rx - R, 0, P.w - 1);
        s_src[ry * TW + rx] = P.pk1[(unsigned)(sy * P.pitch + sx)];
    }
    __syncthreads();
    const int x = x0 + threadIdx.x, y = y0 + threadIdx.y;
    if (x >= P.w || y >= P.h) return;
    const float fvx = flow[(y * P.w + x) * 2], fvy = flow[(y * P.w + x) * 2 + 1];
    if (c2f_unknown(fvx, fvy)) {
        if (SPLIT == 0) c2f_store_flow(flow, y * P.w + x, 0, 0);
        return;
    }
    const int ccx = c2f_centre(fvx, x), ccy = c2f_centre(fvy, y);
    const rgbf c1 = texel_rgb(s_src[(threadIdx.y + R) * TW + threadIdx.x + R]);
    int bx = ccx, by = ccy;
    float min_cost = 999999;
#pragma unroll 1
    for (int m = 0; m < 3; m++) {
        if (SPLIT == 3 && m != m_only) continue;
        const int cx = (int)(int16_t)(ccx + m - 1);
        if (cx < 0 || cx >= P.w) continue;
        rgbf c2[3];
#pragma unroll
        for (int n = 0; n < 3; n++) c2[n] = texel_rgb(tex_px(P.pk2, P.pitch, P.w, P.h, cx, ccy + n - 1));
        float run[3];
        const int cx16 = cx << 4, wmax16 = (P.w - 1) << 4;
        if (SPLIT == 4) {
            if (part == 3) c2f_pass<R, 3, true>(P, L, s_src, TW, threadIdx.x, threadIdx.y, cx16, wmax16, ccy, c1, c2, run);
            else if (part == 2) c2f_pass<R, 2, true>(P, L, s_src, TW, threadIdx.x, threadIdx.y, cx16, wmax16, ccy, c1, c2, run);
            else if (part == 1) c2f_pass<R, 1, true>(P, L, s_src, TW, threadIdx.x, threadIdx.y, cx16, wmax16, ccy, c1, c2, run);
            else c2f_pass<R, 0, true>(P, L, s_src, TW, threadIdx.x, threadIdx.y, cx16, wmax16, ccy, c1, c2, run);
#pragma unroll
            for (int n = 0; n < 3; n++) cost9[(size_t)(y * P.w + x) * 36 + part * 9 + m * 3 + n] = run[n];
            continue;
        }
        c2f_pass<R, 3>(P, L, s_src, TW, threadIdx.x, threadIdx.y, cx16, wmax16, ccy, c1, c2, run);
        c2f_pass<R, 2>(P, L, s_src, TW, threadIdx.x, threadIdx.y, cx16, wmax16, ccy, c1, c2, run);
        c2f_pass<R, 1>(P, L, s_src, TW, threadIdx.x, threadIdx.y, cx16, wmax16, ccy, c1, c2, run);
        c2f_pass<R, 0>(P, L, s_src, TW, threadIdx.x, threadIdx.y, cx16, wmax16, ccy, c1, c2, run);
        if (SPLIT == 3) {
#pragma unroll
            for (int n = 0; n < 3; n++) cost9[(size_t)(y * P.w + x) * 36 + m * 3 + n] = run[n];
            continue;
        }
#pragma unroll
        for (int n = 0; n < 3; n++) {
            const int cy = (int)(int16_t)(ccy + n - 1);
            if (cy < 0 || cy >= P.h) continue;
            const float cv = run[n];
            if (cv < min_cost) { min_cost = cv; bx = cx; by = cy; }
        }
    }
    if (SPLIT != 0) return;
    flow[(y * P.w + x) * 2] = (float)(bx - x);
    flow[(y * P.w + x) * 2 + 1] = (float)(by - y);
}

template <int R, bool PROBE = false>
__global__ __launch_bounds__(512) __attribute__((amdgpu_waves_per_eu(EPPM_C2F_WIN_WAVES, EPPM_C2F_WIN_WAVES)))
void k_c2f_refine_win(PlanesH Ph, float* __restrict__ flow_, const float* __restrict__ lut, size_t pstride, int pre, unsigned* __restrict__ stat,
                      float* __restrict__ probe)
{
    using W = C2fWinShape<R>;
    constexpr int TWU = C2fSrcTile<R>::TWU, TW = C2fSrcTile<R>::TW, WW = W::WW, WH = W::WH;
    static_assert(TWU * TW * 16 >= 9 * 256 * 4, "the exchange buffer aliases the source tile");
    __shared__ EPPM_LUT_ALIGN PatchLutT<R + 1> L;
    __shared__ float4 s_src[TWU * TW];
    __shared__ float4 s_win[WH * WW];
    __shared__ int s_mm[4];
#ifndef EPPM_TOL
    __shared__ int s_pre[1];
#endif
    float* __restrict__ flow = pair_ptr(flow_, pstride, blockIdx.y);
    const int ptid = threadIdx.y * kBlock + threadIdx.x;
    const int grp = threadIdx.z;
    const int tid = grp * 256 + ptid;
    load_patch_lut<EPPM_C2F_LOG2>(L, lut, R, tid, 512);
    const Planes P = to_dev(Ph, pstride, blockIdx.y);
    const uint32_t* __restrict__ pc1 = pair_ptr_opt(Ph.pc1, pstride, blockIdx.y);
    const uint32_t* __restrict__ pc2 = pair_ptr_opt(Ph.pc2, pstride, blockIdx.y);
    int x0, y0, part;
    if (!c2f_tile_origin<0>(P, x0, y0, part)) return;
    if (tid == 0) { s_mm[0] = 0x7fffffff; s_mm[1] = -0x7fffffff; s_mm[2] = 0x7fffffff; s_mm[3] = -0x7fffffff; }
#ifndef EPPM_TOL
    if (tid == 0) s_pre[0] = 0;
#endif
    for (int t = tid; t < TWU * TWU; t += 512) {
        const int ry = t / TWU, rx = t % TWU;
        const int sy = iclamp(y0 + ry - R, 0, P.h - 1), sx = iclamp(x0 + rx - R, 0, P.w - 1);
        s_src[ry * TW + rx] = stage_texel(pc1, P.pk1, (unsigned)(sy * P.pitch + sx));
    }
    __syncthreads();
    const int x = x0 + threadIdx.x, y = y0 + threadIdx.y;
    const bool inimg = (x < P.w && y < P.h);
    float fvx = 0.0f, fvy = 0.0f;
    if (inimg) { fvx = flow[(y * P.w + x) * 2]; fvy = flow[(y * P.w + x) * 2 + 1]; }
    const bool known = inimg && !(fvx > kUnknownFlowThresh || fvy > kUnknownFlowThresh);
    const int ccx = c2f_centre(fvx, x), ccy = c2f_centre(fvy, y);
    if (known && grp == 0) {
        atomicMin(&s_mm[0], ccx); atomicMax(&s_mm[1], ccx);
        atomicMin(&s_mm[2], ccy); atomicMax(&s_mm[3], ccy);
    }
    __syncthreads();
    const int mnx = s_mm[0], mxx = s_mm[1], mny = s_mm[2], mxy = s_mm[3];
    const bool coherent = (mxx - mnx <= W::SPAN_X) && (mxy - mny <= W::SPAN_Y);
    const int wx0 = mnx - 1 + W::XLO, wy0 = mny - 1 + W::YLO;
    if (coherent && mxx >= mnx) {
        for (int t = tid; t < WH * WW; t += 512) {
            const int sy = iclamp(wy0 + t / WW, 0, P.h - 1), sx = iclamp(wx0 + t % WW, 0, P.w - 1);
            s_win[t] = stage_texel(pc2, P.pk2, (unsigned)(sy * P.pitch + sx));
        }
    }
    __syncthreads();
#ifndef EPPM_TOL
    int path = 3;
    if (pre && coherent && mxx >= mnx) {
        constexpr int S = R + 1, I0 = (S - EPPM_C2F_PRE_ROWS) / 2, I1 = I0 + EPPM_C2F_PRE_ROWS;
        constexpr int PADB = C2fPreList<R>::PADB, KROWS = C2fPreList<R>::KROWS, CAP = C2fPreList<R>::CAP;
        static_assert(PADB % 8 == 0 && PADB > 0 && KROWS < TWU, "keys and items do not straddle a row's padding");
        auto pad = [&](int o) -> char* { return reinterpret_cast<char*>(s_src) + (o / PADB) * (TW * 16) + TWU * 16 + (o % PADB); };
        auto key_at = [&](int p) -> unsigned long long* { return reinterpret_cast<unsigned long long*>(pad(p * 8)); };
        auto item_at = [&](int i) -> uint16_t* { return reinterpret_cast<uint16_t*>(pad(KROWS * PADB + i * 2)); };
        const int lane = tid & 63;
        float N[18], D[18], U = 0.0f;
        unsigned vmask = 0;
        rgbf c1 = {0.0f, 0.0f, 0.0f};
        if (known) {
            c1 = texel_rgb(s_src[(threadIdx.y + R) * TW + threadIdx.x + R]);
#pragma unroll 1
            for (int ii = 0; ii < S; ii++) {
                if (ii >= I0 && ii < I1) continue;
                const float4* __restrict__ srow = s_src + (threadIdx.y + 2 * ii) * TW + threadIdx.x;
#pragma unroll
                for (int jj = 0; jj < S; jj++) U += rest_weight_term(c1, srow[2 * jj], L.gsp[ii * S + jj]);
            }
        }
#pragma unroll
        for (int m = 0; m < 3; m++) {
            const int cx = (int)(int16_t)(ccx + m - 1);
            float cs[6] = {0.0f, 0.0f, 0.0f, 0.0f, 0.0f, 0.0f}, ws[6] = {0.0f, 0.0f, 0.0f, 0.0f, 0.0f, 0.0f};
            if (known && !(cx < 0 || cx >= P.w)) {
                const int wbase = ((ccy - 1 - wy0) * WW + (cx - wx0)) * 16;
                rgbf c2[3];
#pragma unroll
                for (int n = 0; n < 3; n++) {
                    c2[n] = texel_rgb(*reinterpret_cast<const float4*>(reinterpret_cast<const char*>(s_win) + wbase + n * (WW * 16)));
                    const int cy = (int)(int16_t)(ccy + n - 1);
                    if (!(cy < 0 || cy >= P.h)) vmask |= 1u << (m * 3 + n);
                }
                if (grp == 0) c2f_rows2_win<R, 3, 2, WW, I0, I1, 3>(L, s_src, TW, threadIdx.x, threadIdx.y, c1, c2, s_win, wbase, cs, ws);
                else c2f_rows2_win<R, 1, 0, WW, I0, I1, 3>(L, s_src, TW, threadIdx.x, threadIdx.y, c1, c2, s_win, wbase, cs, ws);
            }
#pragma unroll
            for (int n = 0; n < 3; n++) { N[m * 3 + n] = cs[n]; D[m * 3 + n] = ws[n]; N[9 + m * 3 + n] = cs[3 + n]; D[9 + m * 3 + n] = ws[3 + n]; }
        }
        if (PROBE && known) {
            float* __restrict__ pp = probe + ((size_t)blockIdx.y * P.h * P.w + (size_t)y * P.w + x) * 73;
            const int qa = (grp == 0 ? 3 : 1) * 9, qb = (grp == 0 ? 2 : 0) * 9;
#pragma unroll
            for (int k = 0; k < 9; k++) { pp[qa + k] = N[k]; pp[36 + qa + k] = D[k]; pp[qb + k] = N[9 + k]; pp[36 + qb + k] = D[9 + k]; }
            if (grp == 1) pp[72] = U;
        }
        bool small = false;
#pragma unroll
        for (int k = 0; k < 9; k++)
            if ((vmask >> k) & 1) small = small || !(D[k] > EPPM_C2F_PRE_DMIN) || !(D[9 + k] > EPPM_C2F_PRE_DMIN);
        if (small) s_pre[0] = 1;
        if (grp == 1) {
            int ks = 15;
            float e_best = 0.0f;
#pragma unroll
            for (int k = 0; k < 9; k++) {
                if (!((vmask >> k) & 1)) continue;
                const float e = c2f_min(N[k] / D[k], N[9 + k] / D[9 + k]);
                if (ks == 15 || e < e_best) { e_best = e; ks = k; }
            }
            *key_at(ptid) = 0xfffffffffffffff0ull | (unsigned)ks;
        }
        __syncthreads();
        path = 1;
        if (!s_pre[0]) {
            const int ks = (int)(*reinterpret_cast<const uint32_t*>(key_at(ptid)) & 15u);
            const bool live = known && ks != 15;
            if (live) {
                const int cx = (int)(int16_t)(ccx + ks / 3 - 1);
                const int wbase = ((ccy - 1 + ks % 3 - wy0) * WW + (cx - wx0)) * 16;
                const rgbf c2[1] = {texel_rgb(*reinterpret_cast<const float4*>(reinterpret_cast<const char*>(s_win) + wbase))};
                float cs[2], ws[2];
                if (grp == 0) c2f_rows2_win<R, 3, 2, WW, 0, S, 1>(L, s_src, TW, threadIdx.x, threadIdx.y, c1, c2, s_win, wbase, cs, ws);
                else c2f_rows2_win<R, 1, 0, WW, 0, S, 1>(L, s_src, TW, threadIdx.x, threadIdx.y, c1, c2, s_win, wbase, cs, ws);
                const float c = c2f_min(cs[0] / ws[0], cs[1] / ws[1]);
                atomicMin(key_at(ptid), ((unsigned long long)__float_as_uint(c) << 4) | (unsigned)ks);
            }
            __syncthreads();
            unsigned sa = 0, sb = 0, tested = 0;
            if (live) {
                const float B = __uint_as_float((uint32_t)(*key_at(ptid) >> 4));
#pragma unroll
                for (int k = 0; k < 9; k++) {
                    if (!((vmask >> k) & 1) || k == ks) continue;
                    const float ra = B * (D[k] + U), rb = B * (D[9 + k] + U);
                    if (!(N[k] * (1.0f - EPPM_C2F_PRE_EPS) >= ra && ra >= EPPM_C2F_PRE_RHSMIN)) sa |= 1u << k;
                    if (!(N[9 + k] * (1.0f - EPPM_C2F_PRE_EPS) >= rb && rb >= EPPM_C2F_PRE_RHSMIN)) sb |= 1u << k;
                    tested += 2;
                }
            }
            const int na = __popc(sa), nb = __popc(sb);
            int ia = na, ib = nb;
#pragma unroll
            for (int d = 1; d < 64; d <<= 1) {
                const int ta = __shfl_up(ia, d), tb = __shfl_up(ib, d);
                if (lane >= d) { ia += ta; ib += tb; }
            }
            static_assert(KROWS * PADB >= 256 * 8 + 16 * 4, "the counts follow the keys");
            auto qcnt_at = [&](int i) -> int* { return reinterpret_cast<int*>(pad(256 * 8 + i * 4)); };
            const int wq = __builtin_amdgcn_readfirstlane((tid >> 6) & 3);
            if (lane == 63) { *qcnt_at(wq * 4 + (grp == 0 ? 3 : 1)) = ia; *qcnt_at(wq * 4 + (grp == 0 ? 2 : 0)) = ib; }
            if (stat && tested) { atomicAdd(stat + 4, tested); atomicAdd(stat + 5, tested - (unsigned)(na + nb)); }
// ... 254 lines not shown
    int bx = ccx, by = ccy;
    float min_cost = 999999;
#pragma unroll
    for (int m = 0; m < 3; m++) {
        const int cx = (int)(int16_t)(ccx + m - 1);
        if (cx < 0 || cx >= P.w) continue;
#pragma unroll
        for (int n = 0; n < 3; n++) {
            const int cy = (int)(int16_t)(ccy + n - 1);
            if (cy < 0 || cy >= P.h) continue;
            const int k = m * 3 + n;
            const float c_4 = res[k], c_3 = xch[k * 256 + ptid], c_2 = xch[(9 + k) * 256 + ptid], c_1 = xch[(18 + k) * 256 + ptid];
            const float cv = c2f_min4(c_1, c_2, c_3, c_4);
            if (cv < min_cost) { min_cost = cv; bx = cx; by = cy; }
        }
    }
    flow[(y * P.w + x) * 2] = (float)(bx - x);
    flow[(y * P.w + x) * 2 + 1] = (float)(by - y);
}

template <int SPLIT>
__global__ __launch_bounds__(256) void k_c2f_select(float* __restrict__ flow_, const float* __restrict__ cost9_, int w, int h, size_t pstride)
{
    float* __restrict__ flow = pair_ptr(flow_, pstride, blockIdx.z);
    const float* __restrict__ cost9 = pair_ptr(cost9_, pstride, blockIdx.z);
    const int x = blockIdx.x * blockDim.x + threadIdx.x, y = blockIdx.y * blockDim.y + threadIdx.y;
    if (x >= w || y >= h) return;
    const float fvx = flow[(y * w + x) * 2], fvy = flow[(y * w + x) * 2 + 1];
    if (c2f_unknown(fvx, fvy)) { c2f_store_flow(flow, y * w + x, 0, 0); return; }
    c2f_select_best(flow, x, y, c2f_centre(fvx, x), c2f_centre(fvy, y), w, h, [=](int m, int n) {
        const float* __restrict__ pc = cost9 + (size_t)(y * w + x) * 36 + m * 3 + n;
        float cv = pc[0];
        if (SPLIT == 4) {
            cv = pc[27];
            cv = c2f_min(pc[18], cv);
            cv = c2f_min(pc[9], cv);
            cv = c2f_min(pc[0], cv);
        }
        return cv;
    });
}

bool c2f_window_span(int R, int* span_x, int* span_y)
{
    if (!(R == 9 || R == 17)) return false;
    *span_x = (R == 9) ? C2fWinShape<9>::SPAN_X : C2fWinShape<17>::SPAN_X;
    *span_y = (R == 9) ? C2fWinShape<9>::SPAN_Y : C2fWinShape<17>::SPAN_Y;
    return true;
}

void c2f_pretest_knobs(int R, int* on, int* row0, int* rows, int* cap, int* parts, float* eps, float* dmin, float* rhsmin)
{
#ifdef EPPM_TOL
    *on = 0;
#else
    *on = EPPM_C2F_PRE;
#endif
    *row0 = (R + 1 - EPPM_C2F_PRE_ROWS) / 2; *rows = EPPM_C2F_PRE_ROWS;
    *cap = C2fPreList<9>::CAP;
    *parts = EPPM_C2F_PRE_PARTS;
    *eps = EPPM_C2F_PRE_EPS; *dmin = EPPM_C2F_PRE_DMIN; *rhsmin = EPPM_C2F_PRE_RHSMIN;
}

static bool c2f_table_ok(int w, int h, int R) { return (w + R < 32764) && (h + R < 32764); }

int c2f_refine_split_factor(int w, int h, int R, int npairs, bool no_split)
{
    if (no_split || !(R == 9 || R == 17) || !c2f_table_ok(w, h, R)) return 0;
    const int tiles = ((w + kBlock - 1) / kBlock) * ((h + kBlock - 1) / kBlock);
    if (!(tiles * npairs * 4 < EPPM_C2F_SPLIT_BELOW_WAVES)) return 0;
    auto imbalance = [&](int f) { const int wgs = tiles * f * npairs; return (float)((wgs + 255) / 256) * 256.0f / (float)wgs; };
    return (imbalance(4) < imbalance(3)) ? 4 : 3;
}
bool c2f_refine_wants_split(int w, int h, int R, int npairs, bool no_split) { return c2f_refine_split_factor(w, h, R, npairs, no_split) != 0; }

template <class F>
static void with_radius(int R, F&& f)
{
    if (R == 9) f(std::integral_constant<int, 9>{});
    else f(std::integral_constant<int, 17>{});
}

void launch_c2f_refine(const PlanesH& P, float* flow, const float* lut, int R, float* cost9, hipStream_t s, Batch bt, bool no_split, int pre,
                       unsigned* stat, float* probe)
{
    dim3 grid((P.w + kBlock - 1) / kBlock, (P.h + kBlock - 1) / kBlock, bt.n), block(kBlock, kBlock);
    const int per_xcd = (grid.x * grid.y + 7) / 8;
    dim3 grid1(per_xcd * 8, bt.n);
    const int f = cost9 ? c2f_refine_split_factor(P.w, P.h, R, bt.n, no_split) : 0;
    launch_note(kLaunchRefine, P.w, P.h, bt.n, f, R);
    if (f) {
        dim3 gridf(per_xcd * f * 8, bt.n), gs((P.w + 63) / 64, (P.h + 3) / 4, bt.n), bs(64, 4);
        with_radius(R, [&](auto r) {
            if (f == 3) hipLaunchKernelGGL((k_c2f_refine_tiled<r(), 3>), gridf, block, 0, s, P, flow, lut, cost9, bt.stride);
            else hipLaunchKernelGGL((k_c2f_refine_tiled<r(), 4>), gridf, block, 0, s, P, flow, lut, cost9, bt.stride);
        });
        if (f == 3) hipLaunchKernelGGL(k_c2f_select<3>, gs, bs, 0, s, flow, cost9, P.w, P.h, bt.stride);
        else hipLaunchKernelGGL(k_c2f_select<4>, gs, bs, 0, s, flow, cost9, P.w, P.h, bt.stride);
        return;
    }
    if (!(R == 9 || R == 17) || !c2f_table_ok(P.w, P.h, R)) {
        hipLaunchKernelGGL(k_c2f_refine, grid, block, 0, s, P, flow, lut, R, bt.stride);
        return;
    }
    const bool window = (R == 9) ? EPPM_C2F_WINDOW : EPPM_C2F_WINDOW17;
    if (!window) with_radius(R, [&](auto r) { hipLaunchKernelGGL((k_c2f_refine_tiled<r(), 0>), grid1, block, 0, s, P, flow, lut, (float*)nullptr, bt.stride); });
    else if (R == 9 && probe) hipLaunchKernelGGL((k_c2f_refine_win<9, true>), grid1, dim3(kBlock, kBlock, 2), 0, s, P, flow, lut, bt.stride, 1, stat, probe);
    else if (R == 9) hipLaunchKernelGGL((k_c2f_refine_win<9>), grid1, dim3(kBlock, kBlock, 2), 0, s, P, flow, lut, bt.stride, pre < 0 ? EPPM_C2F_PRE : pre, stat, (float*)nullptr);
    else hipLaunchKernelGGL((k_c2f_refine_win4<17>), grid1, dim3(kBlock, kBlock, 4), 0, s, P, flow, lut, bt.stride);
}

}
```

### eppm_amd/csrc/k_flow_blf.hip

```cpp
#include <type_traits>

#include "eppm_device.cuh"
#include "eppm_internal.h"

#ifndef EPPM_BLF_UNROLL
#define EPPM_BLF_UNROLL 21
#endif
#ifndef EPPM_BLF_MIX
#define EPPM_BLF_MIX 3
#endif
#ifndef EPPM_BLF_MIX1
#define EPPM_BLF_MIX1 2
#endif
#ifdef EPPM_BLF_WAVES
#define EPPM_BLF_OCC __attribute__((amdgpu_waves_per_eu(EPPM_BLF_WAVES, EPPM_BLF_WAVES)))
#else
#define EPPM_BLF_OCC
#endif
#define EPPM_BLF_PRAGMA_(x) _Pragma(#x)
#define EPPM_BLF_UNROLL_PRAGMA(n) EPPM_BLF_PRAGMA_(unroll n)

namespace eppm {

constexpr int BT_W = 32, BR = kBlfRadius, BTW = BT_W + 2 * BR;
template <int PPL>
__device__ __forceinline__ constexpr bool blf_by_formula(int dx, int pixel)
{
    constexpr int M = (PPL == 1) ? EPPM_BLF_MIX1 : EPPM_BLF_MIX;
    return M == 1 ? (PPL == 2 ? pixel == 1 : (dx & 1)) : M >= 2 ? dx % M == 0 : false;
}
template <int PPL>
__global__ __launch_bounds__(256) EPPM_BLF_OCC void k_flow_blf(float* __restrict__ out_, const float* __restrict__ in_,
                                                  const uint32_t* __restrict__ img_, int ipitch, int w, int h, int fpitch,
                                                  const float* __restrict__ blf_lut, size_t pstride)
{
    float* __restrict__ out = pair_ptr(out_, pstride, blockIdx.z);
    const float* __restrict__ in = pair_ptr(in_, pstride, blockIdx.z);
    const uint32_t* __restrict__ img = pair_ptr(img_, pstride, blockIdx.z);
    constexpr int BT_H = 8 * PPL, BTH = BT_H + 2 * BR;
    __shared__ float4 s_t[BTH * BTW];
    __shared__ float s_fy[BTH * BTW];
    __shared__ float s_lut[BR + 1];
    __shared__ DeltaTab s_D;
    const int x0 = blockIdx.x * BT_W, y0 = blockIdx.y * BT_H;
    const int tid = threadIdx.y * BT_W + threadIdx.x;
    if (tid <= BR) s_lut[tid] = blf_lut[tid];
    load_delta_tab<false>(s_D, blf_lut + BR + 1, tid, 256);
    for (int t = tid; t < BTW * BTH; t += 256) {
        const int cy = y0 + t / BTW - BR, cx = x0 + t % BTW - BR;
        float4 e = make_float4(100.0f, 0.0f, 0.0f, 0.0f);
        float fy = 0.0f;
        if (cx >= 0 && cy >= 0 && cx < w && cy < h) {
            e.w = in[(cy * fpitch + cx) * 2];
            fy = in[(cy * fpitch + cx) * 2 + 1];
            if (!(e.w > kUnknownFlowThresh || fy > kUnknownFlowThresh)) {
                const rgbf c = unpack_rgb(img[cy * ipitch + cx]);
                e.x = c.x; e.y = c.y; e.z = c.z;
            }
        }
        s_t[t] = e;
        s_fy[t] = fy;
    }
    __syncthreads();
    const int x = x0 + threadIdx.x, ya = y0 + PPL * threadIdx.y;
    if (x >= w || ya >= h) return;
    const bool has_b = (PPL == 2) && (ya + 1 < h);
    const rgbf ca = unpack_rgb(img[ya * ipitch + x]);
    const rgbf cb = unpack_rgb(img[(has_b ? ya + 1 : ya) * ipitch + x]);
    float nxa = 0.f, nya = 0.f, wa = 0.f, nxb = 0.f, nyb = 0.f, wb = 0.f;
    const int base = (PPL * threadIdx.y) * BTW + threadIdx.x;
    auto tap_row = [&](int r, auto use_a, auto use_b) {
        const float gya = use_a ? s_lut[abs(r - BR)] : 0.0f;
        const float gyb = use_b ? s_lut[abs(r - 1 - BR)] : 0.0f;
EPPM_BLF_UNROLL_PRAGMA(EPPM_BLF_UNROLL)
        for (int dx = 0; dx <= 2 * BR; dx++) {
            const int ti = base + r * BTW + dx;
            const float4 tp = s_t[ti];
            const float tfy = s_fy[ti];
            const rgbf pix = {tp.x, tp.y, tp.z};
            const float gx = s_lut[abs(dx - BR)];
            if (use_a) {
                const bool tab_a = EPPM_DELTA_BLF && !blf_by_formula<PPL>(dx, 0);
                const float delta_r = tab_a ? __builtin_amdgcn_fmed3f(max_abs_diff(ca, pix), 0.0f, 1.0f) : max_abs_diff(ca, pix);
                const float coef_r = tab_a ? delta_lookup_off(s_D, delta_r) : fast_exp(div_wmf2(-(delta_r * delta_r)));
                const float coef_s = gx * gya;
                const float wgt = coef_r * coef_s;
                nxa += wgt * tp.w;
                nya += wgt * tfy;
                wa += wgt;
            }
            if (use_b) {
                const bool tab_b = EPPM_DELTA_BLF && !blf_by_formula<PPL>(dx, 1);
                const float delta_r = tab_b ? __builtin_amdgcn_fmed3f(max_abs_diff(cb, pix), 0.0f, 1.0f) : max_abs_diff(cb, pix);
                const float coef_r = tab_b ? delta_lookup_off(s_D, delta_r) : fast_exp(div_wmf2(-(delta_r * delta_r)));
                const float coef_s = gx * gyb;
                const float wgt = coef_r * coef_s;
                nxb += wgt * tp.w;
                nyb += wgt * tfy;
                wb += wgt;
            }
        }
    };
    if (PPL == 2) {
        tap_row(0, std::true_type{}, std::false_type{});
#pragma unroll 1
        for (int r = 1; r <= 2 * BR; r++) tap_row(r, std::true_type{}, std::true_type{});
        tap_row(2 * BR + 1, std::false_type{}, std::true_type{});
    } else {
#pragma unroll 1
        for (int r = 0; r <= 2 * BR; r++) tap_row(r, std::true_type{}, std::false_type{});
    }
    {
        const int ci = base + BR * BTW + BR;
        float ox = s_t[ci].w, oy = s_fy[ci];
        if (wa != 0) { ox = nxa / wa; oy = nya / wa; }
        out[(ya * fpitch + x) * 2] = ox;
        out[(ya * fpitch + x) * 2 + 1] = oy;
    }
    if (has_b) {
        const int ci = base + (BR + 1) * BTW + BR;
        float ox = s_t[ci].w, oy = s_fy[ci];
        if (wb != 0) { ox = nxb / wb; oy = nyb / wb; }
        out[((ya + 1) * fpitch + x) * 2] = ox;
        out[((ya + 1) * fpitch + x) * 2 + 1] = oy;
    }
}
int flow_blf_pixels_per_lane(int w, int h, int npairs)
{
    const int wgs2 = ((w + BT_W - 1) / BT_W) * ((h + 15) / 16) * npairs;
    return wgs2 >= 8 * 256 ? 2 : 1;
}
void launch_flow_blf(float* out, const float* in, const uint32_t* img, int ipitch, int w, int h, int flow_pitch,
                     const float* blf_lut, hipStream_t s, Batch bt)
{
    dim3 block(BT_W, 8);
    const int ppl = flow_blf_pixels_per_lane(w, h, bt.n);
    launch_note(kLaunchSmoothing, w, h, bt.n, ppl);
    if (ppl == 2) {
        hipLaunchKernelGGL(k_flow_blf<2>, dim3((w + BT_W - 1) / BT_W, (h + 15) / 16, bt.n), block, 0, s, out, in, img, ipitch, w, h, flow_pitch, blf_lut, bt.stride);
    } else {
        hipLaunchKernelGGL(k_flow_blf<1>, dim3((w + BT_W - 1) / BT_W, (h + 7) / 8, bt.n), block, 0, s, out, in, img, ipitch, w, h, flow_pitch, blf_lut, bt.stride);
    }
}

}
```

### eppm_amd/csrc/k_prepare.hip

```cpp
#include "eppm_device.cuh"
#include "eppm_internal.h"

namespace eppm {

constexpr int GT_W = 32, GT_H = 8, G_MAXR = 6;

__global__ __launch_bounds__(256) void k_gauss_rgba(uint32_t* __restrict__ out0, const uint32_t* __restrict__ in0,
                                                    uint32_t* __restrict__ out1, const uint32_t* __restrict__ in1, int pitch,
                                                    int h, int w, float sigma2, int radius, int nimg, size_t pstride)
{
    const unsigned pair = blockIdx.z / nimg, im = blockIdx.z % nimg;
    uint32_t* __restrict__ out = pair_ptr(im ? out1 : out0, pstride, pair);
    const uint32_t* __restrict__ in = pair_ptr(im ? in1 : in0, pstride, pair);
    __shared__ uint32_t tile[(GT_H + 2 * G_MAXR) * (GT_W + 2 * G_MAXR)];
    __shared__ float wtab[(2 * G_MAXR + 1) * (2 * G_MAXR + 1)];
    const int tw = GT_W + 2 * radius, th = GT_H + 2 * radius;
    const int x0 = blockIdx.x * GT_W, y0 = blockIdx.y * GT_H;
    const int tid = threadIdx.y * GT_W + threadIdx.x;
    for (int t = tid; t < tw * th; t += 256) {
        const int ty = t / tw, tx = t % tw;
        const int cy = max(0, min(h - 1, y0 + ty - radius));
        const int cx = max(0, min(w - 1, x0 + tx - radius));
        tile[t] = in[cy * pitch + cx];
    }
    const int d = 2 * radius + 1;
    for (int t = tid; t < d * d; t += 256) {
        const int dy = t / d - radius, dx = t % d - radius;
        wtab[t] = fast_exp(-(float)(dy * dy + dx * dx) / sigma2);
    }
    __syncthreads();
    const int x = x0 + threadIdx.x, y = y0 + threadIdx.y;
    if (x >= w || y >= h) return;
    float vx = 0, vy = 0, vz = 0, vw = 0, sum = 0;
    for (int dy = 0; dy < d; dy++)
        for (int dx = 0; dx < d; dx++) {
            const float weight = wtab[dy * d + dx];
            const uint32_t p = tile[(threadIdx.y + dy) * tw + threadIdx.x + dx];
            vx += (float)(p & 0xffu) * weight;
            vy += (float)((p >> 8) & 0xffu) * weight;
            vz += (float)((p >> 16) & 0xffu) * weight;
            vw += (float)(p >> 24) * weight;
            sum += weight;
        }
    vx /= sum; vy /= sum; vz /= sum; vw /= sum;
    const uint32_t r = (uint32_t)vx | ((uint32_t)vy << 8) | ((uint32_t)vz << 16) | ((uint32_t)vw << 24);
    out[y * pitch + x] = r;
}

void launch_gauss_rgba(uint32_t* out, const uint32_t* in, int pitch_px, int h, int w, float sigma, int radius, hipStream_t s, Batch bt)
{
    dim3 grid((w + GT_W - 1) / GT_W, (h + GT_H - 1) / GT_H, bt.n), block(GT_W, GT_H);
    hipLaunchKernelGGL(k_gauss_rgba, grid, block, 0, s, out, in, out, in, pitch_px, h, w, sigma * sigma * 2, radius, 1, bt.stride);
}
void launch_gauss_rgba2(uint32_t* out0, const uint32_t* in0, uint32_t* out1, const uint32_t* in1, int pitch_px, int h, int w, float sigma,
                        int radius, hipStream_t s, Batch bt)
{
    dim3 grid((w + GT_W - 1) / GT_W, (h + GT_H - 1) / GT_H, 2 * bt.n), block(GT_W, GT_H);
    hipLaunchKernelGGL(k_gauss_rgba, grid, block, 0, s, out0, in0, out1, in1, pitch_px, h, w, sigma * sigma * 2, radius, 2, bt.stride);
}

__global__ __launch_bounds__(256) void k_gauss_decimate2(uint32_t* __restrict__ out0, const uint32_t* __restrict__ in0,
                                                         uint32_t* __restrict__ out1, const uint32_t* __restrict__ in1, int out_pitch,
                                                         int outH, int outW, int pitch, int h, int w, float sigma2, int radius, int nimg,
                                                         size_t pstride)
{
    const unsigned pair = blockIdx.z / nimg, im = blockIdx.z % nimg;
    uint32_t* __restrict__ out = pair_ptr(im ? out1 : out0, pstride, pair);
    const uint32_t* __restrict__ in = pair_ptr(im ? in1 : in0, pstride, pair);
    __shared__ uint32_t tile[(2 * GT_H + 2 * G_MAXR) * (2 * GT_W + 2 * G_MAXR)];
    __shared__ float wtab[(2 * G_MAXR + 1) * (2 * G_MAXR + 1)];
    const int tw = 2 * GT_W + 2 * radius, th = 2 * GT_H + 2 * radius;
    const int x0 = blockIdx.x * GT_W, y0 = blockIdx.y * GT_H;
    const int sx0 = 2 * x0 + 1 - radius, sy0 = 2 * y0 + 1 - radius;
    const int tid = threadIdx.y * GT_W + threadIdx.x;
    for (int t = tid; t < tw * th; t += 256) {
        const int ty = t / tw, tx = t % tw;
        const int cy = max(0, min(h - 1, sy0 + ty));
        const int cx = max(0, min(w - 1, sx0 + tx));
        tile[t] = in[cy * pitch + cx];
    }
    const int d = 2 * radius + 1;
    for (int t = tid; t < d * d; t += 256) {
        const int dy = t / d - radius, dx = t % d - radius;
        wtab[t] = fast_exp(-(float)(dy * dy + dx * dx) / sigma2);
    }
    __syncthreads();
    const int x = x0 + threadIdx.x, y = y0 + threadIdx.y;
    if (x >= outW || y >= outH) return;
    const int lx = 2 * threadIdx.x, ly = 2 * threadIdx.y;
    float vx = 0, vy = 0, vz = 0, vw = 0, sum = 0;
    for (int dy = 0; dy < d; dy++)
        for (int dx = 0; dx < d; dx++) {
            const float weight = wtab[dy * d + dx];
            const uint32_t p = tile[(ly + dy) * tw + lx + dx];
            vx += (float)(p & 0xffu) * weight;
            vy += (float)((p >> 8) & 0xffu) * weight;
            vz += (float)((p >> 16) & 0xffu) * weight;
            vw += (float)(p >> 24) * weight;
            sum += weight;
        }
    vx /= sum; vy /= sum; vz /= sum; vw /= sum;
    out[y * out_pitch + x] = (uint32_t)vx | ((uint32_t)vy << 8) | ((uint32_t)vz << 16) | ((uint32_t)vw << 24);
}

bool gauss_decimate2_ok(int outH, int outW, int h, int w, float ratio, int radius)
{
    return ratio == 0.5f && radius <= G_MAXR && 2 * (outW - 1) + 1 <= w - 1 && 2 * (outH - 1) + 1 <= h - 1;
}
void launch_gauss_decimate2(uint32_t* out0, const uint32_t* in0, uint32_t* out1, const uint32_t* in1, int nimg, int out_pitch_px, int outH,
                            int outW, int pitch_px, int h, int w, float sigma, int radius, hipStream_t s, Batch bt)
{
    dim3 grid((outW + GT_W - 1) / GT_W, (outH + GT_H - 1) / GT_H, nimg * bt.n), block(GT_W, GT_H);
    hipLaunchKernelGGL(k_gauss_decimate2, grid, block, 0, s, out0, in0, out1, in1, out_pitch_px, outH, outW, pitch_px, h, w,
                       sigma * sigma * 2, radius, nimg, bt.stride);
}

__global__ __launch_bounds__(256) void k_resize_rgba(uint32_t* __restrict__ out_, int out_pitch, int outH, int outW,
                                                     const uint32_t* __restrict__ in_, int in_pitch, int h, int w, float ratio, size_t pstride)
{
    uint32_t* __restrict__ out = pair_ptr(out_, pstride, blockIdx.z);
    const uint32_t* __restrict__ in = pair_ptr(in_, pstride, blockIdx.z);
    const int x = blockIdx.x * blockDim.x + threadIdx.x, y = blockIdx.y * blockDim.y + threadIdx.y;
    if (x >= outW || y >= outH) return;
    const float div_scale = 1.f / ratio;
    const float fx = (float)(x + 1) * div_scale - 1;
    const float fy = (float)(y + 1) * div_scale - 1;
    const int xx = (int)fx, yy = (int)fy;
    const float dx = fmaxf(fminf(fx - xx, 1), 0);
    const float dy = fmaxf(fminf(fy - yy, 1), 0);
// ... 167 lines not shown
```

### eppm_amd/csrc/launchers_ref_abi.cpp

```cpp
#include "stage_object.h"
#include "mblur.h"

using namespace eppm;

namespace {
struct DevState {
    float *lut_pm = nullptr, *lut_wmf = nullptr, *lut_blf = nullptr;
    int lut_R = -1;
    void* scratch[9] = {nullptr, nullptr, nullptr, nullptr, nullptr, nullptr, nullptr, nullptr, nullptr};
    size_t scratch_bytes[9] = {0, 0, 0, 0, 0, 0, 0, 0, 0};
    std::map<std::tuple<int, int, int, unsigned long long>, eppm_pm_rng*> rngs;
};
std::mutex g_mu;
std::map<int, DevState> g_dev;
hipStream_t g_stream = nullptr;
eppm_params g_prm = {9, 10, 30, 6, 10, 20, 1234ULL, 0, kNumLevels};
int g_launch_status = EPPM_OK;

int dev_state(DevState** out)
{
    int d = 0;
    HIPCHK(hipGetDevice(&d));
    DevState& s = g_dev[d];
    if (s.lut_R != g_prm.patch_r) {
// ... 360 lines not shown
                              ds->lut_wmf, num_iter, is_only_occlusion ? 1 : 0, (uint32_t*)ws, g_stream);
    if (res != (int16_t*)d_disp_vec && (g_launch_status = copy_d2d(d_disp_vec, res, disp_pitch * h)) != EPPM_OK) return;
    g_launch_status = finish();
}

extern "C" void baoCudaFillHole(eppm_short2* d_disp_vec, float* d_cost, eppm_uchar4* d_img, int w, int h,
        size_t img_pitch, size_t cost_pitch, size_t disp_pitch)
{
    (void)d_cost; (void)cost_pitch;
    LAUNCHER_BEGIN;
    void* tmp = nullptr;
    g_launch_status = get_scratch(ds, disp_pitch * h, &tmp);
    if (g_launch_status != EPPM_OK) return;
    if ((g_launch_status = copy_d2d(tmp, d_disp_vec, disp_pitch * h)) != EPPM_OK) return;
    launch_fill_holes((int16_t*)d_disp_vec, (const int16_t*)tmp, (const uint32_t*)d_img, (int)(img_pitch / 4), w, h, (int)(disp_pitch / 4), g_stream);
    g_launch_status = finish();
}

extern "C" void baoCudaNNF2Flow(eppm_float2* d_flow, eppm_short2* d_disp_vec, int w, int h, size_t disp_pitch, size_t flow_pitch)
{
    std::lock_guard<std::mutex> lk(g_mu);
    launch_nnf2flow((float*)d_flow, (int)(flow_pitch / 8), (const int16_t*)d_disp_vec, (int)(disp_pitch / 4), w, h, g_stream);
    g_launch_status = finish();
}

extern "C" void baoCudaBLFCostFilterRefine(eppm_float2* d_flow_vec, eppm_uchar4* d_img1, eppm_uchar4* d_img2, unsigned char* d_census1,
        unsigned char* d_census2, int w, int h, size_t img_pitch, size_t census_pitch)
{
    LAUNCHER_BEGIN;
    PlanesH P;
    g_launch_status = mk_planes(ds, &P, d_img1, d_img2, d_census1, d_census2, w, h, img_pitch, census_pitch);
    if (g_launch_status != EPPM_OK) return;
    float* cost9 = nullptr;
    if ((g_launch_status = split_scratch(ds, w, h, &cost9)) != EPPM_OK) return;
    launch_c2f_refine(P, (float*)d_flow_vec, ds->lut_pm, g_prm.patch_r, cost9, g_stream, kOnePair, opt_no_split() != 0, opt_c2f_pre());
    g_launch_status = finish();
}

extern "C" void baoCudaBLF_C2F(eppm_float2** pFlowPyr, eppm_uchar4** pImgPyr1, eppm_uchar4** pImgPyr2, unsigned char** pCensusPyr1,
        unsigned char** pCensusPyr2, eppm_float2** pTempPyr1, eppm_float2** pTempPyr2, int* arrH, int* arrW,
        size_t* arrPitchUchar4, size_t* arrPitchUchar1, int nLayerIdx)
{
    (void)pTempPyr1; (void)pTempPyr2;
    LAUNCHER_BEGIN;
    const int l = nLayerIdx;
    launch_resize_flow((float*)pFlowPyr[l], arrH[l], arrW[l], (const float*)pFlowPyr[l + 1], arrH[l + 1], arrW[l + 1], 2.0f, 1.0f, g_stream);
    launch_mul_scalar((float*)pFlowPyr[l], 2.0f, arrH[l], arrW[l], g_stream);
    PlanesH P;
    g_launch_status = mk_planes(ds, &P, pImgPyr1[l], pImgPyr2[l], pCensusPyr1[l], pCensusPyr2[l], arrW[l], arrH[l], arrPitchUchar4[l], arrPitchUchar1[l]);
    if (g_launch_status != EPPM_OK) return;
    float* cost9 = nullptr;
    if ((g_launch_status = split_scratch(ds, arrW[l], arrH[l], &cost9)) != EPPM_OK) return;
    launch_c2f_refine(P, (float*)pFlowPyr[l], ds->lut_pm, g_prm.patch_r, cost9, g_stream, kOnePair, opt_no_split() != 0, opt_c2f_pre());
    g_launch_status = finish();
}

#ifdef EPPM_TEST_HOOKS
static int c2f_refine_batch(float* d_flow, const uint32_t* d_img1, const uint32_t* d_img2, const uint8_t* d_census1,
        const uint8_t* d_census2, int w, int h, int npairs, int pre, unsigned* stat, float* d_probe = nullptr)
{
#ifdef EPPM_TOL
    if (pre == 1 || d_probe) return set_err(EPPM_ERR_ARG, "the tolerance library's window refine has no two-phase form");
#endif
    if (!d_flow || !d_img1 || !d_img2 || !d_census1 || !d_census2 || w < 1 || h < 1 || npairs < 1)
        return set_err(EPPM_ERR_ARG, "eppm_test_c2f_refine_batch: bad argument");
    LAUNCHER_BEGIN_INT;
    const size_t n = (size_t)w * h, stride = n * 16;
    void *a = nullptr, *b = nullptr, *f = nullptr, *st = nullptr;
    CHK(get_scratch(ds, stride * npairs, &a, 2));
    CHK(get_scratch(ds, stride * npairs, &b, 3));
    CHK(get_scratch(ds, stride * npairs + 32, &f, 0));
    if (stat) {
        st = (char*)f + stride * npairs;
        HIPCHK(hipMemsetAsync(st, 0, 32, g_stream));
    }
    for (int p = 0; p < npairs; p++) {
        launch_pack((char*)a + p * stride, w, d_img1 + p * n, w, d_census1 + p * n, w, w, h, g_stream);
        launch_pack((char*)b + p * stride, w, d_img2 + p * n, w, d_census2 + p * n, w, w, h, g_stream);
        CHK(copy_d2d((char*)f + p * stride, d_flow + p * n * 2, n * 8));
    }
    PlanesH P;
    P.pk1 = a; P.pk2 = b; P.w = w; P.h = h; P.pitch = w;
    if (d_probe) HIPCHK(hipMemsetAsync(d_probe, 0xff, n * npairs * 73 * 4, g_stream));
    launch_c2f_refine(P, (float*)f, ds->lut_pm, g_prm.patch_r, nullptr, g_stream, Batch{npairs, stride}, opt_no_split() != 0, pre, (unsigned*)st, d_probe);
    for (int p = 0; p < npairs; p++) CHK(copy_d2d(d_flow + p * n * 2, (char*)f + p * stride, n * 8));
    if (stat) { HIPCHK(hipMemcpyAsync(stat, st, 32, hipMemcpyDeviceToHost, g_stream)); HIPCHK(hipStreamSynchronize(g_stream)); }
    return finish();
}
extern "C" int eppm_test_c2f_refine_batch(float* d_flow, const uint32_t* d_img1, const uint32_t* d_img2, const uint8_t* d_census1,
        const uint8_t* d_census2, int w, int h, int npairs)
{
    return c2f_refine_batch(d_flow, d_img1, d_img2, d_census1, d_census2, w, h, npairs, opt_c2f_pre(), nullptr);
}
extern "C" int eppm_test_c2f_refine_pre(float* d_flow, const uint32_t* d_img1, const uint32_t* d_img2, const uint8_t* d_census1,
        const uint8_t* d_census2, int w, int h, int npairs, int pre, unsigned* stat)
{
    if (!stat || pre < -1 || pre > 1) return set_err(EPPM_ERR_ARG, "eppm_test_c2f_refine_pre: bad argument");
    return c2f_refine_batch(d_flow, d_img1, d_img2, d_census1, d_census2, w, h, npairs, pre, stat);
}
extern "C" int eppm_test_c2f_refine_probe(float* d_flow, const uint32_t* d_img1, const uint32_t* d_img2, const uint8_t* d_census1,
        const uint8_t* d_census2, int w, int h, int npairs, float* d_probe)
{
    if (!d_probe || g_prm.patch_r != 9) return set_err(EPPM_ERR_ARG, "eppm_test_c2f_refine_probe: bad argument (patch radius 9 only)");
    return c2f_refine_batch(d_flow, d_img1, d_img2, d_census1, d_census2, w, h, npairs, 1, nullptr, d_probe);
}
#endif

#ifdef EPPM_TEST_HOOKS
extern "C" int eppm_test_pm_search(eppm_pm_rng* r, float* d_cost, eppm_short2* d_nnf, const uint32_t* d_img1, const uint32_t* d_img2, int w, int h,
                                   int ndir, int npairs, int pretest, float* d_restw, float* d_pre_n, float* d_pre_d)
{
    if (!r || !d_cost || !d_nnf || !d_img1 || !d_img2 || w != r->w || h != r->h || ndir < 1 || ndir > 2 || npairs < 1)
        return set_err(EPPM_ERR_ARG, "eppm_test_pm_search: bad argument");
    LAUNCHER_BEGIN_INT;
    const int R = g_prm.patch_r;
    if (r->G != g_prm.num_guess || (R != 9 && R != 17)) return set_err(EPPM_ERR_ARG, "eppm_test_pm_search: num_guess %d / patch_r %d", r->G, R);
    const size_t n = (size_t)w * h;
    const int pad = (R + 2) & ~1, ppitch = parity_pitch(w, pad);
    size_t off = 0;
    auto carve = [&](size_t bytes) { const size_t o = off; off = (off + bytes + 255) & ~(size_t)255; return o; };
    size_t o_img[2], o_cen[2], o_pk[2], o_pc[2], o_pp[2], o_cost[2], o_nnf[2], o_rw[2], o_pn[2], o_pd[2];
    for (int k = 0; k < 2; k++) { o_img[k] = carve(n * 4); o_cen[k] = carve(n); o_pk[k] = carve(n * 16); o_pc[k] = carve(n * 4); o_pp[k] = carve((size_t)2 * h * ppitch * 4); }
    for (int k = 0; k < ndir; k++) { o_cost[k] = carve(n * 4); o_nnf[k] = carve(n * 4); o_rw[k] = carve(n * 4); o_pn[k] = carve(n * 4); o_pd[k] = carve(n * 4); }
    const size_t stride = (off + 4095) & ~(size_t)4095;
    void *slab = nullptr, *tab = nullptr;
    CHK(get_scratch(ds, stride * npairs, &slab, 0));
    CHK(get_scratch(ds, (size_t)r->gx * r->gy * 512 * r->G * sizeof(int16_t), &tab, 7));
    char* S = (char*)slab;
    for (int p = 0; p < npairs; p++) {
        CHK(copy_d2d(S + p * stride + o_img[0], d_img1 + p * n, n * 4));
        CHK(copy_d2d(S + p * stride + o_img[1], d_img2 + p * n, n * 4));
        for (int k = 0; k < ndir; k++) {
            CHK(copy_d2d(S + p * stride + o_cost[k], d_cost + (p * ndir + k) * n, n * 4));
            CHK(copy_d2d(S + p * stride + o_nnf[k], (const char*)d_nnf + (p * ndir + k) * n * 4, n * 4));
        }
    }
    const Batch bt{npairs, stride};
    CensusBatch cb;
    cb.n = 2;
    for (int k = 0; k < 2; k++) {
        CensusJob& J = cb.job[k];
        J.census = (uint8_t*)(S + o_cen[k]); J.cpitch = w; J.texels = S + o_pk[k]; J.tpitch = w; J.img = (const uint32_t*)(S + o_img[k]); J.ipitch = w;
        J.w = w; J.h = h; J.first_block = 0; J.packed = (uint32_t*)(S + o_pc[k]);
    }
    launch_census_batch(cb, g_stream, bt);
    for (int k = 0; k < 2; k++) launch_parity_planes((uint32_t*)(S + o_pp[k]), ppitch, pad, (const uint32_t*)(S + o_pc[k]), w, w, h, g_stream, bt);
    PmBatch b;
    b.n = ndir; b.cpitch = w; b.npitch = w; b.npairs = npairs; b.stride = stride;
    for (int k = 0; k < ndir; k++) {
        PlanesH P;
        P.pk1 = S + o_pk[k]; P.pk2 = S + o_pk[k ^ 1]; P.w = w; P.h = h; P.pitch = w;
        P.pc1 = (const uint32_t*)(S + o_pc[k]); P.pc2 = (const uint32_t*)(S + o_pc[k ^ 1]);
        P.pp1 = (const uint32_t*)(S + o_pp[k]); P.pp2 = (const uint32_t*)(S + o_pp[k ^ 1]); P.pp_pitch = ppitch; P.pp_pad = pad;
        b.p[k] = mk_problem(P, (float*)(S + o_cost[k]), (int16_t*)(S + o_nnf[k]), nullptr, nullptr, 0, nullptr, nullptr, nullptr, nullptr, (float*)(S + o_rw[k]));
    }
    PmRngDev d = r->dev();
    launch_pm_rand_table(d, r->work[0][r->cur[0]], (int16_t*)tab, r->G, g_stream);
    d.rand_tab = (const int16_t*)tab;
    if (pretest) {
        if (!pm_search_pretest_ready(b, d, R)) return set_err(EPPM_ERR_ARG, "eppm_test_pm_search: no two-phase search at patch_r %d", R);
        launch_pm_rest_weight(b, ds->lut_pm, R, g_stream);
        if (d_pre_n && d_pre_d) {
            PmPretestSums ps{};
            for (int k = 0; k < ndir; k++) { ps.n[k] = (float*)(S + o_pn[k]); ps.d[k] = (float*)(S + o_pd[k]); }
            launch_pm_pretest_probe(b, ds->lut_pm, R, ps, g_stream);
        }
    }
    launch_pm_random_search(b, d, ds->lut_pm, R, g_prm.search_range, g_prm.num_guess, g_stream, pretest != 0);
    for (int p = 0; p < npairs; p++)
        for (int k = 0; k < ndir; k++) {
            CHK(copy_d2d(d_cost + (p * ndir + k) * n, S + p * stride + o_cost[k], n * 4));
            CHK(copy_d2d((char*)d_nnf + (p * ndir + k) * n * 4, S + p * stride + o_nnf[k], n * 4));
            if (pretest && d_restw) CHK(copy_d2d(d_restw + (p * ndir + k) * n, S + p * stride + o_rw[k], n * 4));
            if (pretest && d_pre_n && d_pre_d) {
                CHK(copy_d2d(d_pre_n + (p * ndir + k) * n, S + p * stride + o_pn[k], n * 4));
                CHK(copy_d2d(d_pre_d + (p * ndir + k) * n, S + p * stride + o_pd[k], n * 4));
            }
        }
    return finish();
}
#endif

extern "C" void baoCudaFlowSmoothing(eppm_float2* d_flow, eppm_uchar4* d_img, int w, int h, size_t img_pitch, size_t flow_pitch)
{
    LAUNCHER_BEGIN;
    void* tmp = nullptr;
    g_launch_status = get_scratch(ds, flow_pitch * h, &tmp);
// ... 131 lines not shown
```

### eppm_amd/stages.py

```python
import ctypes as C

import numpy as np

from ._lib import CParams, check, check_launcher, lib, probe_dispatch
from .api import float2, short2, uchar4


class Dev:

    def __init__(self, arr=None, shape=None, dtype=None, pitched=False):
        if arr is not None:
            arr = np.ascontiguousarray(arr)
            shape, dtype = arr.shape, arr.dtype
        self.h, self.w = shape
        self.dtype = np.dtype(dtype)
        row = self.w * self.dtype.itemsize
        self.ptr = C.c_void_p()
        if pitched:
            pitch = C.c_size_t()
            check(lib().eppm_malloc_pitched(C.byref(self.ptr), C.byref(pitch), C.c_size_t(row), C.c_size_t(self.h)), "malloc_pitched")
            self.pitch = pitch.value
        else:
            check(lib().eppm_malloc_device(C.byref(self.ptr), C.c_size_t(row * self.h)), "malloc")
            self.pitch = row
# ... 218 lines not shown
    lib().baoCudaOutlierRemoval(a.ptr, b.ptr, w, h, _sz(b.pitch), _sz(a.pitch))
    check_launcher("baoCudaOutlierRemoval")
    return a.get(), b.get()


def weighted_median(nnf, img, num_iter=20, only_occlusion=True):
    h, w = nnf.shape
    a, i = Dev(nnf), Dev(img, pitched=True)
    lib().baoCudaWeightedMedianFilter(a.ptr, None, i.ptr, w, h, _sz(i.pitch), _sz(w * 4), _sz(a.pitch), num_iter, C.c_bool(only_occlusion))
    check_launcher("baoCudaWeightedMedianFilter")
    return a.get()


def fill_holes(nnf, img):
    h, w = nnf.shape
    a, i = Dev(nnf), Dev(img, pitched=True)
    lib().baoCudaFillHole(a.ptr, None, i.ptr, w, h, _sz(i.pitch), _sz(w * 4), _sz(a.pitch))
    check_launcher("baoCudaFillHole")
    return a.get()


def nnf2flow(nnf):
    h, w = nnf.shape
    a, f = Dev(nnf), Dev(shape=(h, w), dtype=float2)
    lib().baoCudaNNF2Flow(f.ptr, a.ptr, w, h, _sz(a.pitch), _sz(f.pitch))
    check_launcher("baoCudaNNF2Flow")
    return f.get()


def resize_flow(flow, out_h, out_w, ratio=2.0):
    h, w = flow.shape
    a, b = Dev(flow), Dev(shape=(out_h, out_w), dtype=float2)
    check(lib().eppm_resize_flow(b.ptr, out_h, out_w, a.ptr, h, w, C.c_float(ratio)), "resize_flow")
    return b.get()


def flow_upsample(coarse, img):
    h, w = img.shape
    hc, wc = coarse.shape
    a, i, b = Dev(coarse), Dev(img, pitched=True), Dev(shape=(h, w), dtype=float2)
    check(lib().eppm_flow_upsample(b.ptr, h, w, a.ptr, hc, wc, i.ptr, _sz(i.pitch)), "eppm_flow_upsample")
    return b.get()


def c2f_refine(flow, P):
    f = Dev(flow)
    lib().baoCudaBLFCostFilterRefine(f.ptr, *P.args(), P.w, P.h, _sz(P.i1.pitch), _sz(P.c1.pitch))
    check_launcher("baoCudaBLFCostFilterRefine")
    return f.get()


def c2f_refine_batch(flows, planes):
    n = len(flows)
    h, w = flows[0].shape
    f = Dev(np.concatenate([np.ascontiguousarray(x, float2) for x in flows]))
    i1, i2, c1, c2 = (Dev(np.concatenate([np.ascontiguousarray(p[k]) for p in planes])) for k in range(4))
    check(lib().eppm_test_c2f_refine_batch(f.ptr, i1.ptr, i2.ptr, c1.ptr, c2.ptr, w, h, n), "eppm_test_c2f_refine_batch")
    out = f.get()
    return [out[k * h:(k + 1) * h] for k in range(n)]


def c2f_refine_pre(flows, planes, pre, parts=False):
    n = len(flows)
    h, w = flows[0].shape
    f = Dev(np.concatenate([np.ascontiguousarray(x, float2) for x in flows]))
    i1, i2, c1, c2 = (Dev(np.concatenate([np.ascontiguousarray(p[k]) for p in planes])) for k in range(4))
    stat = (C.c_uint * 8)()
    check(lib().eppm_test_c2f_refine_pre(f.ptr, i1.ptr, i2.ptr, c1.ptr, c2.ptr, w, h, n, int(pre), stat), "eppm_test_c2f_refine_pre")
    out = f.get()
    return [out[k * h:(k + 1) * h] for k in range(n)], tuple(stat[:8 if parts else 6])


def c2f_refine_probe(flows, planes):
    n = len(flows)
    h, w = flows[0].shape
    f = Dev(np.concatenate([np.ascontiguousarray(x, float2) for x in flows]))
    i1, i2, c1, c2 = (Dev(np.concatenate([np.ascontiguousarray(p[k]) for p in planes])) for k in range(4))
    pr = Dev(shape=(n * h, w * 73), dtype=np.float32)
    check(lib().eppm_test_c2f_refine_probe(f.ptr, i1.ptr, i2.ptr, c1.ptr, c2.ptr, w, h, n, pr.ptr), "eppm_test_c2f_refine_probe")
    out, p = f.get(), pr.get().reshape(n, h, w, 73)
    return [out[k * h:(k + 1) * h] for k in range(n)], p[..., :36].reshape(n, h, w, 4, 9), p[..., 36:72].reshape(n, h, w, 4, 9), p[..., 72]


def probe_c2f_pretest(patch_r=9):
    out, fl = _c2f_pretest_knobs(patch_r)
    return bool(out[0]), out[1], out[2], out[3], fl[0], fl[1], fl[2]


def probe_c2f_parts(patch_r=9):
    return bool(_c2f_pretest_knobs(patch_r)[0][4])


def _c2f_pretest_knobs(patch_r):
    out = (C.c_int * 5)()
    fl = (C.c_float * 3)()
    check(lib().eppm_probe_c2f_pretest(patch_r, out, fl), "eppm_probe_c2f_pretest")
    return out, fl


def blf_c2f(flow_coarse, P_fine, coarse_dims):
    ch, cw = coarse_dims
    fine = Dev(shape=(P_fine.h, P_fine.w), dtype=float2)
    coarse = Dev(flow_coarse)
    tab = lambda a, b: (C.c_void_p * 2)(a, b)
    arrH = (C.c_int * 2)(P_fine.h, ch)
    arrW = (C.c_int * 2)(P_fine.w, cw)
    p4 = (C.c_size_t * 2)(P_fine.i1.pitch, 0)
    pc = (C.c_size_t * 2)(P_fine.c1.pitch, 0)
    lib().baoCudaBLF_C2F(tab(fine.ptr, coarse.ptr), tab(P_fine.i1.ptr, None), tab(P_fine.i2.ptr, None), tab(P_fine.c1.ptr, None),
                         tab(P_fine.c2.ptr, None), None, None, arrH, arrW, p4, pc, 0)
    check_launcher("baoCudaBLF_C2F")
    return fine.get()


def flow_smoothing(flow, img):
    h, w = flow.shape
    f, i = Dev(flow), Dev(img, pitched=True)
    lib().baoCudaFlowSmoothing(f.ptr, i.ptr, w, h, _sz(i.pitch), _sz(f.pitch))
    check_launcher("baoCudaFlowSmoothing")
    return f.get()


def temporal_prior(prev, backward=False):
    d_prev = Dev(np.ascontiguousarray(prev, short2))
    d_out = Dev(shape=prev.shape, dtype=short2)
    check(lib().eppm_temporal_prior(d_out.ptr, d_prev.ptr, d_prev.h, d_prev.w, int(bool(backward))), "eppm_temporal_prior")
    check(lib().eppm_device_synchronize(), "eppm_device_synchronize")
    return d_out.get()


def temporal_prior_batch(prevs, backward=False, armed=None, calls=1):
    prevs = np.ascontiguousarray(prevs, short2)
    n, h, w = prevs.shape
    d_prev = Dev(prevs.reshape(n * h, w))
    d_out = Dev(shape=(n * h, w), dtype=short2)
    flags = None if armed is None else (C.c_uint8 * n)(*[int(bool(x)) for x in armed])
    out = []
    for _ in range(calls):
        check(lib().eppm_temporal_prior_batch(d_out.ptr, d_prev.ptr, h, w, int(bool(backward)), n, flags), "eppm_temporal_prior_batch")
        check(lib().eppm_device_synchronize(), "eppm_device_synchronize")
        out.append(d_out.get().reshape(n, h, w))
    return out[0] if calls == 1 else out


def flow_to_color(flow, max_disp_x=20.0, max_disp_y=20.0):
    h, w = flow.shape
    f, c = Dev(flow), Dev(shape=(h, w), dtype=uchar4)
    check(lib().eppm_flow_to_color(c.ptr, f.ptr, h, w, C.c_float(max_disp_x), C.c_float(max_disp_y)), "eppm_flow_to_color")
    return c.get()
```

Before: 255.3 Mflow-vectors/s.

## Split c2f rest-weight into its own pass and stream device I/O directly

Three separate changes. First, the per-pixel rest-weight sum in the coarse-to-fine refine window kernel moves into a separate kernel that writes a float plane, which the refine kernel then reads instead of recomputing it, lowering register and ALU pressure in the heavy window kernel at the cost of an extra launch and a plane round-trip. Second, device-resident input frames are read directly by a new Gaussian prefilter kernel that also writes the raw copy, replacing the two hipMemcpy2DAsync calls. Third, the final flow bilateral filter writes straight into the caller's output buffers, removing the device-to-device copy.

```diff
diff --git a/eppm_amd/_lib.py b/eppm_amd/_lib.py
--- a/eppm_amd/_lib.py
+++ b/eppm_amd/_lib.py
@@ -170,7 +170,7 @@
 ]
 
 
-TEST_SYMBOLS = ["eppm_test_set_option", "eppm_test_c2f_refine_batch", "eppm_test_c2f_refine_pre", "eppm_test_c2f_refine_probe", "eppm_probe_c2f_pretest", "eppm_probe_c2f_window", "eppm_probe_dispatch", "eppm_probe_fast_exp", "eppm_probe_div_const", "eppm_probe_delta_table",
+TEST_SYMBOLS = ["eppm_test_set_option", "eppm_test_c2f_refine_batch", "eppm_test_c2f_refine_pre", "eppm_test_c2f_refine_probe", "eppm_test_c2f_rest_weight", "eppm_probe_c2f_pretest", "eppm_probe_c2f_window", "eppm_probe_dispatch", "eppm_probe_fast_exp", "eppm_probe_div_const", "eppm_probe_delta_table",
                 "eppm_probe_unpack_texel", "eppm_probe_pm_parity", "eppm_probe_ctx_rng_states", "eppm_test_pm_search", "eppm_probe_search_pretest", "eppm_probe_launch_log"]
 
 _variant = None
@@ -225,7 +225,7 @@
     check(lib().eppm_launcher_status(), what)
 
 
-LAUNCH_STAGES = ("smoothing", "jbu", "refine", "search", "sweep", "sweeps_merged")
+LAUNCH_STAGES = ("smoothing", "jbu", "refine", "search", "sweep", "sweeps_merged", "rest_weight")
 
 
 class launch_log:
diff --git a/eppm_amd/csrc/api_internal.h b/eppm_amd/csrc/api_internal.h
--- a/eppm_amd/csrc/api_internal.h
+++ b/eppm_amd/csrc/api_internal.h
@@ -63,6 +63,8 @@
 static inline int opt_search_pre() { return g_opt_search_pre.load(); }
 EPPM_HIDDEN extern std::atomic<int> g_opt_c2f_pre;
 static inline int opt_c2f_pre() { return g_opt_c2f_pre.load(); }
+EPPM_HIDDEN extern std::atomic<int> g_opt_c2f_restw;
+static inline int opt_c2f_restw() { return g_opt_c2f_restw.load(); }
 EPPM_HIDDEN extern std::atomic<int> g_opt_alloc_fill;
 static inline int opt_alloc_fill() { return g_opt_alloc_fill.load(); }
 EPPM_HIDDEN hipError_t alloc_fill(hipError_t e, void* p, size_t bytes, bool pinned);
@@ -73,6 +75,7 @@
 static constexpr int opt_force_split() { return 0; }
 static constexpr int opt_search_pre() { return -1; }
 static constexpr int opt_c2f_pre() { return -1; }
+static constexpr int opt_c2f_restw() { return -1; }
 static constexpr int opt_alloc_fill() { return -1; }
 #endif
 
diff --git a/eppm_amd/csrc/c2f_device.cuh b/eppm_amd/csrc/c2f_device.cuh
--- a/eppm_amd/csrc/c2f_device.cuh
+++ b/eppm_amd/csrc/c2f_device.cuh
@@ -35,6 +35,9 @@
 #endif
 #ifndef EPPM_C2F_PRE_PARTS
 #define EPPM_C2F_PRE_PARTS 1
+#endif
+#ifndef EPPM_C2F_U_PLANE
+#define EPPM_C2F_U_PLANE 1
 #endif
 #define EPPM_C2F_PRE_DMIN 0x1p-60f
 #define EPPM_C2F_PRE_RHSMIN 0x1p-100f
diff --git a/eppm_amd/csrc/context.cpp b/eppm_amd/csrc/context.cpp
--- a/eppm_amd/csrc/context.cpp
+++ b/eppm_amd/csrc/context.cpp
@@ -117,7 +117,7 @@
     HIPCHK(hipSetDevice(device));
     eppm_ctx* c = new eppm_ctx();
     c->device = device; c->prm = p; c->h = h; c->w = w; c->npairs = npairs; c->n_active = 1;
-    c->opt_sweep_spec = opt_sweep_spec(); c->opt_no_split = opt_no_split(); c->opt_search_pre = opt_search_pre(); c->opt_c2f_pre = opt_c2f_pre();
+    c->opt_sweep_spec = opt_sweep_spec(); c->opt_no_split = opt_no_split(); c->opt_search_pre = opt_search_pre(); c->opt_c2f_pre = opt_c2f_pre(); c->opt_c2f_restw = opt_c2f_restw();
     c->nl = pyr_init_dim(c->H, c->W, h, w, p.levels, 0.5f);
     const int L = c->nl - 1;
     if (c->H[L] < 1 || c->W[L] < 1 || (c->W[L] + p.seg_len - 1) / p.seg_len > 1024 || (c->H[L] + p.seg_len - 1) / p.seg_len > 1024) {
diff --git a/eppm_amd/csrc/context.h b/eppm_amd/csrc/context.h
--- a/eppm_amd/csrc/context.h
+++ b/eppm_amd/csrc/context.h
@@ -10,7 +10,7 @@
     int device = 0;
     hipStream_t stream = nullptr;
     bool own_stream = false;
-    int opt_sweep_spec = -1, opt_no_split = 0, opt_search_pre = -1, opt_c2f_pre = -1;
+    int opt_sweep_spec = -1, opt_no_split = 0, opt_search_pre = -1, opt_c2f_pre = -1, opt_c2f_restw = -1;
     eppm_params prm;
     int h = 0, w = 0, nl = 0;
     int stop_level = 0;
@@ -50,6 +50,7 @@
     hipEvent_t ev_h2d = nullptr;
     int rgb_cur = 0;
     float* h_flow = nullptr;
+    const eppm::FlowOuts* direct_out = nullptr;
     std::vector<float*> out_u, out_v;
     eppm::HostHold out_hold;
     bool have_images = false, have_flow = false;
diff --git a/eppm_amd/csrc/ctx_compute.cpp b/eppm_amd/csrc/ctx_compute.cpp
--- a/eppm_amd/csrc/ctx_compute.cpp
+++ b/eppm_amd/csrc/ctx_compute.cpp
@@ -96,7 +96,9 @@
     hipStream_t s = c->stream;
     const Batch bt = c->bt();
     const int L = c->nl - 1;
-    auto blf = [&](float* dst, const float* src, int l) { launch_flow_blf(dst, src, d.guide[l], (int)(c->ipitch[l] / 4), c->W[l], c->H[l], c->W[l], c->lut_blf, s, bt); };
+    auto blf = [&](float* dst, const float* src, int l, const FlowOuts* outs = nullptr) {
+        launch_flow_blf(dst, src, d.guide[l], (int)(c->ipitch[l] / 4), c->W[l], c->H[l], c->W[l], c->lut_blf, s, bt, outs);
+    };
     const int stop = c->stop_level;
     float* r = d.a[L];
     for (int l = L - 1; l >= 0; l--) {
@@ -113,7 +115,13 @@
         launch_resize_flow(d.a[l], c->H[l], c->W[l], r, c->H[l + 1], c->W[l + 1], 2.0f, 2.0f, s, bt);
         stage_end(c, c->ev);
         stage_begin(c, c->ev, level_stage.s[kStageRefine][d.bwd][l], d.dominant);
-        launch_c2f_refine(planes(c, l, d.swap), d.a[l], c->lut_pm, c->prm.patch_r, c->c2f_cost9[l], s, bt, c->opt_no_split != 0, c->opt_c2f_pre);
+        const PlanesH P = planes(c, l, d.swap);
+        float* restw = nullptr;
+        if (c2f_refine_wants_rest_weight(c->W[l], c->H[l], c->prm.patch_r, bt.n, c->opt_no_split != 0, c->c2f_cost9[l] != nullptr, c->opt_c2f_pre, c->opt_c2f_restw)) {
+            restw = (float*)c->tmpu[l];
+            launch_c2f_rest_weight(P, restw, c->lut_pm, c->prm.patch_r, s, bt);
+        }
+        launch_c2f_refine(P, d.a[l], c->lut_pm, c->prm.patch_r, c->c2f_cost9[l], s, bt, c->opt_no_split != 0, c->opt_c2f_pre, nullptr, nullptr, restw);
         stage_end(c, c->ev, d.dominant);
         stage_begin(c, c->ev, level_stage.s[kStageBlf][d.bwd][l]);
         blf(d.b[l], d.a[l], l);
@@ -124,7 +132,7 @@
     if (stop > 0) return EPPM_OK;
     stage_begin(c, c->ev, d.bwd ? "flow_blf_bwd_final" : "flow_blf_final");
     float* out = (r == d.b[0]) ? d.a[0] : d.b[0];
-    blf(out, r, 0);
+    blf(out, r, 0, d.bwd ? nullptr : c->direct_out);
     CHK(keep(c, 0, out));
     stage_end(c, c->ev);
     return EPPM_OK;
@@ -261,22 +269,32 @@
     return backward_all(c);
 }
 
-extern "C" int eppm_compute_device(eppm_ctx* c, void* d_flow)
-{
-    if (!c) return set_err(EPPM_ERR_ARG, "NULL ctx");
-    CHK(compute_all(c));
-    if (d_flow) HIPCHK(hipMemcpyAsync(d_flow, c->flow[0], (size_t)c->h * c->w * 8, hipMemcpyDeviceToDevice, c->stream));
-    return EPPM_OK;
-}
-
-extern "C" int eppm_batch_compute_device(eppm_ctx* c, void* const* d_flows)
-{
-    if (!c) return set_err(EPPM_ERR_ARG, "NULL ctx");
-    CHK(compute_all(c));
-    if (d_flows)
+static int compute_device(eppm_ctx* c, void* const* d_flows)
+{
+    FlowOuts outs{};
+    bool any = false;
+    for (int k = 0; d_flows && k < c->n_active && k < kFlowOutsMax; k++) { outs.p[k] = (float*)d_flows[k]; any = any || d_flows[k]; }
+    const bool direct = any && flow_direct_out(c->n_active, c->stop_level);
+    c->direct_out = direct ? &outs : nullptr;
+    const int r = compute_all(c);
+    c->direct_out = nullptr;
+    CHK(r);
+    if (d_flows && !direct)
         for (int k = 0; k < c->n_active; k++)
             if (d_flows[k]) HIPCHK(hipMemcpyAsync(d_flows[k], c->of_pair(c->flow[0], k), (size_t)c->h * c->w * 8, hipMemcpyDeviceToDevice, c->stream));
     return EPPM_OK;
+}
+
+extern "C" int eppm_compute_device(eppm_ctx* c, void* d_flow)
+{
+    if (!c) return set_err(EPPM_ERR_ARG, "NULL ctx");
+    return compute_device(c, d_flow ? &d_flow : nullptr);
+}
+
+extern "C" int eppm_batch_compute_device(eppm_ctx* c, void* const* d_flows)
+{
+    if (!c) return set_err(EPPM_ERR_ARG, "NULL ctx");
+    return compute_device(c, d_flows);
 }
 
 static int compute_begin_impl(eppm_ctx* c, int n_out, float* const* u, float* const* v, bool bidir)
diff --git a/eppm_amd/csrc/ctx_images.cpp b/eppm_amd/csrc/ctx_images.cpp
--- a/eppm_amd/csrc/ctx_images.cpp
+++ b/eppm_amd/csrc/ctx_images.cpp
@@ -2,14 +2,15 @@
 
 using namespace eppm;
 
-static int prepare(eppm_ctx* c, bool only2 = false)
+static int prepare(eppm_ctx* c, bool only2 = false, const DirectFrames* direct = nullptr, size_t in_pitch = 0)
 {
     stage_begin(c, c->ev_prep, "prepare");
     hipStream_t s = c->stream;
     const Batch bt = c->bt();
     uint32_t **p1 = c->img1, **p2 = c->img2, **tmp = c->tmpu;
     const int p0 = (int)(c->ipitch[0] / 4);
-    if (only2) launch_gauss_rgba(p2[0], c->raw2, p0, c->H[0], c->W[0], .5f, 2, s, bt);
+    if (direct) launch_gauss_rgba2_direct(p1[0], c->raw1, p2[0], c->raw2, *direct, (int)(in_pitch / 4), p0, c->H[0], c->W[0], .5f, 2, s, bt);
+    else if (only2) launch_gauss_rgba(p2[0], c->raw2, p0, c->H[0], c->W[0], .5f, 2, s, bt);
     else launch_gauss_rgba2(p1[0], c->raw1, p2[0], c->raw2, p0, c->H[0], c->W[0], .5f, 2, s, bt);
     const float ratio = 0.5f;
     const float baseSigma = (1 / ratio - 1);
@@ -137,14 +138,21 @@
 {
     if (pitch < (size_t)c->w * 4 || (pitch & 3)) return set_err(EPPM_ERR_ARG, "eppm_set_images_device: bad pitch %zu", pitch);
     HIPCHK(hipSetDevice(c->device));
-    for (int k = 0; k < n; k++) {
+    for (int k = 0; k < n; k++)
         if (!d1[k] || !d2[k]) return set_err(EPPM_ERR_ARG, "eppm_set_images_device: NULL image");
+    DirectFrames F{};
+    bool direct = prepare_direct_in(n);
+    for (int k = 0; direct && k < n; k++) {
+        F.p[2 * k] = (const uint32_t*)d1[k]; F.p[2 * k + 1] = (const uint32_t*)d2[k];
+        direct = !(((uintptr_t)d1[k] | (uintptr_t)d2[k]) & 3);
+    }
+    for (int k = 0; !direct && k < n; k++) {
         HIPCHK(hipMemcpy2DAsync(c->of_pair(c->raw1, k), c->raw_pitch, d1[k], pitch, (size_t)c->w * 4, c->h, hipMemcpyDeviceToDevice, c->stream));
         HIPCHK(hipMemcpy2DAsync(c->of_pair(c->raw2, k), c->raw_pitch, d2[k], pitch, (size_t)c->w * 4, c->h, hipMemcpyDeviceToDevice, c->stream));
     }
     c->n_active = n;
     c->tmp_drop();
-    return prepare(c);
+    return direct ? prepare(c, false, &F, pitch) : prepare(c);
 }
 
 extern "C" int eppm_set_images_device(eppm_ctx* c, const void* d1, const void* d2, size_t pitch)
diff --git a/eppm_amd/csrc/eppm_internal.h b/eppm_amd/csrc/eppm_internal.h
--- a/eppm_amd/csrc/eppm_internal.h
+++ b/eppm_amd/csrc/eppm_internal.h
@@ -25,7 +25,7 @@
 constexpr Batch kOnePair = {1, 0};
 
 #define EPPM_DECISION __attribute__((visibility("hidden")))
-enum LaunchStage { kLaunchSmoothing = 0, kLaunchJbu, kLaunchRefine, kLaunchSearch, kLaunchSweep, kLaunchSweepsMerged };
+enum LaunchStage { kLaunchSmoothing = 0, kLaunchJbu, kLaunchRefine, kLaunchSearch, kLaunchSweep, kLaunchSweepsMerged, kLaunchRestWeight };
 typedef void (*LaunchNoteFn)(int stage, int w, int h, int npairs, int form, int extra);
 extern EPPM_DECISION std::atomic<LaunchNoteFn> g_launch_note;
 inline void launch_note(int stage, int w, int h, int npairs, int form, int extra = 0)
@@ -162,10 +162,22 @@
 bool c2f_refine_wants_split(int w, int h, int R, int npairs = 1, bool no_split = false);
 bool c2f_window_span(int R, int* span_x, int* span_y);
 void launch_c2f_refine(const PlanesH& P, float* flow, const float* lut, int R, float* cost9, hipStream_t s, Batch bt = kOnePair, bool no_split = false,
-                       int pre = -1, unsigned* stat = nullptr, float* probe = nullptr);
+                       int pre = -1, unsigned* stat = nullptr, float* probe = nullptr, const float* restw = nullptr);
+EPPM_DECISION bool c2f_refine_wants_rest_weight(int w, int h, int R, int npairs, bool no_split, bool has_cost9, int pre, int use = -1);
+void launch_c2f_rest_weight(const PlanesH& P, float* restw, const float* lut, int R, hipStream_t s, Batch bt = kOnePair);
 void c2f_pretest_knobs(int R, int* on, int* row0, int* rows, int* cap, int* parts, float* eps, float* dmin, float* rhsmin);
+#ifndef EPPM_DIRECT_IO
+#define EPPM_DIRECT_IO 1
+#endif
+constexpr int kFlowOutsMax = 8;
+struct FlowOuts { float* p[kFlowOutsMax]; };
+struct DirectFrames { const uint32_t* p[2 * kFlowOutsMax]; };
+EPPM_DECISION bool prepare_direct_in(int npairs);
+void launch_gauss_rgba2_direct(uint32_t* out0, uint32_t* raw0, uint32_t* out1, uint32_t* raw1, const DirectFrames& F, int in_pitch_px, int pitch_px,
+                               int h, int w, float sigma, int radius, hipStream_t s, Batch bt);
 void launch_flow_blf(float* out, const float* in, const uint32_t* img, int ipitch, int w, int h, int flow_pitch,
-                     const float* blf_lut, hipStream_t s, Batch bt = kOnePair);
+                     const float* blf_lut, hipStream_t s, Batch bt = kOnePair, const FlowOuts* outs = nullptr);
+EPPM_DECISION bool flow_direct_out(int npairs, int stop_level);
 EPPM_DECISION int flow_blf_pixels_per_lane(int w, int h, int npairs = 1);
 void launch_flow_jbu(float* out, const float* in_coarse, const uint32_t* img, int ipitch, int w, int h, int wc, int hc, const float* blf_lut,
                      hipStream_t s, Batch bt = kOnePair);
diff --git a/eppm_amd/csrc/k_c2f_refine.hip b/eppm_amd/csrc/k_c2f_refine.hip
--- a/eppm_amd/csrc/k_c2f_refine.hip
+++ b/eppm_amd/csrc/k_c2f_refine.hip
@@ -112,10 +112,51 @@
     flow[(y * P.w + x) * 2 + 1] = (float)(by - y);
 }
 
+#ifndef EPPM_TOL
+template <int R, int I0, int I1>
+__device__ __forceinline__ float c2f_rest_weight(const PatchLutT<R + 1>& L, const float4* __restrict__ s_src, int TW, int tx, int ty, const rgbf c1)
+{
+    constexpr int S = R + 1;
+    float U = 0.0f;
+#pragma unroll 1
+    for (int ii = 0; ii < S; ii++) {
+        if (ii >= I0 && ii < I1) continue;
+        const float4* __restrict__ srow = s_src + (ty + 2 * ii) * TW + tx;
+#pragma unroll
+        for (int jj = 0; jj < S; jj++) U += rest_weight_term(c1, srow[2 * jj], L.gsp[ii * S + jj]);
+    }
+    return U;
+}
+
+template <int R>
+__global__ __launch_bounds__(256) void k_c2f_rest_weight(PlanesH Ph, float* __restrict__ restw_, const float* __restrict__ lut, size_t pstride)
+{
+    constexpr int TWU = C2fSrcTile<R>::TWU, TW = C2fSrcTile<R>::TW, S = R + 1, I0 = (S - EPPM_C2F_PRE_ROWS) / 2, I1 = I0 + EPPM_C2F_PRE_ROWS;
+    __shared__ EPPM_LUT_ALIGN PatchLutT<R + 1> L;
+    __shared__ float4 s_src[TWU * TW];
+    const int tid = threadIdx.y * kBlock + threadIdx.x;
+    load_patch_lut<EPPM_C2F_LOG2>(L, lut, R, tid, 256);
+    const Planes P = to_dev(Ph, pstride, blockIdx.z);
+    const uint32_t* __restrict__ pc1 = pair_ptr_opt(Ph.pc1, pstride, blockIdx.z);
+    float* __restrict__ restw = pair_ptr(restw_, pstride, blockIdx.z);
+    const int x0 = blockIdx.x * kBlock, y0 = blockIdx.y * kBlock;
+    for (int t = tid; t < TWU * TWU; t += 256) {
+        const int ry = t / TWU, rx = t % TWU;
+        const int sy = iclamp(y0 + ry - R, 0, P.h - 1), sx = iclamp(x0 + rx - R, 0, P.w - 1);
+        s_src[ry * TW + rx] = stage_texel(pc1, P.pk1, (unsigned)(sy * P.pitch + sx));
+    }
+    __syncthreads();
+    const int x = x0 + threadIdx.x, y = y0 + threadIdx.y;
+    if (x >= P.w || y >= P.h) return;
+    const rgbf c1 = texel_rgb(s_src[(threadIdx.y + R) * TW + threadIdx.x + R]);
+    restw[y * P.w + x] = c2f_rest_weight<R, I0, I1>(L, s_src, TW, threadIdx.x, threadIdx.y, c1);
+}
+#endif
+
 template <int R, bool PROBE = false>
 __global__ __launch_bounds__(512) __attribute__((amdgpu_waves_per_eu(EPPM_C2F_WIN_WAVES, EPPM_C2F_WIN_WAVES)))
 void k_c2f_refine_win(PlanesH Ph, float* __restrict__ flow_, const float* __restrict__ lut, size_t pstride, int pre, unsigned* __restrict__ stat,
-                      float* __restrict__ probe)
+                      float* __restrict__ probe, const float* __restrict__ restw_)
 {
     using W = C2fWinShape<R>;
     constexpr int TWU = C2fSrcTile<R>::TWU, TW = C2fSrcTile<R>::TW, WW = W::WW, WH = W::WH;
@@ -183,13 +224,9 @@
         rgbf c1 = {0.0f, 0.0f, 0.0f};
         if (known) {
             c1 = texel_rgb(s_src[(threadIdx.y + R) * TW + threadIdx.x + R]);
-#pragma unroll 1
-            for (int ii = 0; ii < S; ii++) {
-                if (ii >= I0 && ii < I1) continue;
-                const float4* __restrict__ srow = s_src + (threadIdx.y + 2 * ii) * TW + threadIdx.x;
-#pragma unroll
-                for (int jj = 0; jj < S; jj++) U += rest_weight_term(c1, srow[2 * jj], L.gsp[ii * S + jj]);
-            }
+            const float* __restrict__ restw = EPPM_C2F_U_PLANE ? pair_ptr_opt(restw_, pstride, blockIdx.y) : nullptr;
+            if (restw) U = restw[y * P.w + x];
+            else U = c2f_rest_weight<R, I0, I1>(L, s_src, TW, threadIdx.x, threadIdx.y, c1);
         }
 #pragma unroll
         for (int m = 0; m < 3; m++) {
@@ -610,7 +647,7 @@
 }
 
 void launch_c2f_refine(const PlanesH& P, float* flow, const float* lut, int R, float* cost9, hipStream_t s, Batch bt, bool no_split, int pre,
-                       unsigned* stat, float* probe)
+                       unsigned* stat, float* probe, const float* restw)
 {
     dim3 grid((P.w + kBlock - 1) / kBlock, (P.h + kBlock - 1) / kBlock, bt.n), block(kBlock, kBlock);
     const int per_xcd = (grid.x * grid.y + 7) / 8;
@@ -633,9 +670,30 @@
     }
     const bool window = (R == 9) ? EPPM_C2F_WINDOW : EPPM_C2F_WINDOW17;
     if (!window) with_radius(R, [&](auto r) { hipLaunchKernelGGL((k_c2f_refine_tiled<r(), 0>), grid1, block, 0, s, P, flow, lut, (float*)nullptr, bt.stride); });
-    else if (R == 9 && probe) hipLaunchKernelGGL((k_c2f_refine_win<9, true>), grid1, dim3(kBlock, kBlock, 2), 0, s, P, flow, lut, bt.stride, 1, stat, probe);
-    else if (R == 9) hipLaunchKernelGGL((k_c2f_refine_win<9>), grid1, dim3(kBlock, kBlock, 2), 0, s, P, flow, lut, bt.stride, pre < 0 ? EPPM_C2F_PRE : pre, stat, (float*)nullptr);
+    else if (R == 9 && probe) hipLaunchKernelGGL((k_c2f_refine_win<9, true>), grid1, dim3(kBlock, kBlock, 2), 0, s, P, flow, lut, bt.stride, 1, stat, probe, restw);
+    else if (R == 9) hipLaunchKernelGGL((k_c2f_refine_win<9>), grid1, dim3(kBlock, kBlock, 2), 0, s, P, flow, lut, bt.stride, pre < 0 ? EPPM_C2F_PRE : pre, stat, (float*)nullptr, restw);
     else hipLaunchKernelGGL((k_c2f_refine_win4<17>), grid1, dim3(kBlock, kBlock, 4), 0, s, P, flow, lut, bt.stride);
 }
 
-}
+bool c2f_refine_wants_rest_weight(int w, int h, int R, int npairs, bool no_split, bool has_cost9, int pre, int use)
+{
+#ifdef EPPM_TOL
+    return false;
+#else
+    if (!(use < 0 ? EPPM_C2F_U_PLANE : (use && EPPM_C2F_U_PLANE))) return false;
+    if (has_cost9 && c2f_refine_split_factor(w, h, R, npairs, no_split)) return false;
+    if (R != 9 || !c2f_table_ok(w, h, R) || !EPPM_C2F_WINDOW) return false;
+    return (pre < 0 ? EPPM_C2F_PRE : pre) != 0;
+#endif
+}
+
+void launch_c2f_rest_weight(const PlanesH& P, float* restw, const float* lut, int R, hipStream_t s, Batch bt)
+{
+#ifndef EPPM_TOL
+    if (R != 9) return;
+    launch_note(kLaunchRestWeight, P.w, P.h, bt.n, 0, R);
+    hipLaunchKernelGGL(k_c2f_rest_weight<9>, dim3((P.w + kBlock - 1) / kBlock, (P.h + kBlock - 1) / kBlock, bt.n), dim3(kBlock, kBlock), 0, s, P, restw, lut, bt.stride);
+#endif
+}
+
+}
diff --git a/eppm_amd/csrc/k_flow_blf.hip b/eppm_amd/csrc/k_flow_blf.hip
--- a/eppm_amd/csrc/k_flow_blf.hip
+++ b/eppm_amd/csrc/k_flow_blf.hip
@@ -30,9 +30,8 @@
     return M == 1 ? (PPL == 2 ? pixel == 1 : (dx & 1)) : M >= 2 ? dx % M == 0 : false;
 }
 template <int PPL>
-__global__ __launch_bounds__(256) EPPM_BLF_OCC void k_flow_blf(float* __restrict__ out_, const float* __restrict__ in_,
-                                                  const uint32_t* __restrict__ img_, int ipitch, int w, int h, int fpitch,
-                                                  const float* __restrict__ blf_lut, size_t pstride)
+__device__ __forceinline__ void flow_blf_tile(float* __restrict__ out_, const float* __restrict__ in_, const uint32_t* __restrict__ img_, int ipitch, int w,
+                                              int h, int fpitch, const float* __restrict__ blf_lut, size_t pstride, float* __restrict__ out2)
 {
     float* __restrict__ out = pair_ptr(out_, pstride, blockIdx.z);
     const float* __restrict__ in = pair_ptr(in_, pstride, blockIdx.z);
@@ -116,6 +115,7 @@
         if (wa != 0) { ox = nxa / wa; oy = nya / wa; }
         out[(ya * fpitch + x) * 2] = ox;
         out[(ya * fpitch + x) * 2 + 1] = oy;
+        if (out2) { out2[(ya * w + x) * 2] = ox; out2[(ya * w + x) * 2 + 1] = oy; }
     }
     if (has_b) {
         const int ci = base + (BR + 1) * BTW + BR;
@@ -123,20 +123,40 @@
         if (wb != 0) { ox = nxb / wb; oy = nyb / wb; }
         out[((ya + 1) * fpitch + x) * 2] = ox;
         out[((ya + 1) * fpitch + x) * 2 + 1] = oy;
+        if (out2) { out2[((ya + 1) * w + x) * 2] = ox; out2[((ya + 1) * w + x) * 2 + 1] = oy; }
     }
+}
+template <int PPL>
+__global__ __launch_bounds__(256) EPPM_BLF_OCC void k_flow_blf(float* __restrict__ out_, const float* __restrict__ in_,
+                                                  const uint32_t* __restrict__ img_, int ipitch, int w, int h, int fpitch,
+                                                  const float* __restrict__ blf_lut, size_t pstride)
+{
+    flow_blf_tile<PPL>(out_, in_, img_, ipitch, w, h, fpitch, blf_lut, pstride, nullptr);
+}
+template <int PPL>
+__global__ __launch_bounds__(256) EPPM_BLF_OCC void k_flow_blf_out(float* __restrict__ out_, const float* __restrict__ in_,
+                                                  const uint32_t* __restrict__ img_, int ipitch, int w, int h, int fpitch,
+                                                  const float* __restrict__ blf_lut, size_t pstride, FlowOuts outs)
+{
+    flow_blf_tile<PPL>(out_, in_, img_, ipitch, w, h, fpitch, blf_lut, pstride, outs.p[blockIdx.z]);
 }
 int flow_blf_pixels_per_lane(int w, int h, int npairs)
 {
     const int wgs2 = ((w + BT_W - 1) / BT_W) * ((h + 15) / 16) * npairs;
     return wgs2 >= 8 * 256 ? 2 : 1;
 }
+bool flow_direct_out(int npairs, int stop_level) { return EPPM_DIRECT_IO && npairs >= 1 && npairs <= kFlowOutsMax && stop_level == 0; }
 void launch_flow_blf(float* out, const float* in, const uint32_t* img, int ipitch, int w, int h, int flow_pitch,
-                     const float* blf_lut, hipStream_t s, Batch bt)
+                     const float* blf_lut, hipStream_t s, Batch bt, const FlowOuts* outs)
 {
     dim3 block(BT_W, 8);
     const int ppl = flow_blf_pixels_per_lane(w, h, bt.n);
-    launch_note(kLaunchSmoothing, w, h, bt.n, ppl);
-    if (ppl == 2) {
+    if (outs && bt.n > kFlowOutsMax) outs = nullptr;
+    launch_note(kLaunchSmoothing, w, h, bt.n, ppl, outs ? 1 : 0);
+    if (outs) {
+        if (ppl == 2) hipLaunchKernelGGL(k_flow_blf_out<2>, dim3((w + BT_W - 1) / BT_W, (h + 15) / 16, bt.n), block, 0, s, out, in, img, ipitch, w, h, flow_pitch, blf_lut, bt.stride, *outs);
+        else hipLaunchKernelGGL(k_flow_blf_out<1>, dim3((w + BT_W - 1) / BT_W, (h + 7) / 8, bt.n), block, 0, s, out, in, img, ipitch, w, h, flow_pitch, blf_lut, bt.stride, *outs);
+    } else if (ppl == 2) {
         hipLaunchKernelGGL(k_flow_blf<2>, dim3((w + BT_W - 1) / BT_W, (h + 15) / 16, bt.n), block, 0, s, out, in, img, ipitch, w, h, flow_pitch, blf_lut, bt.stride);
     } else {
         hipLaunchKernelGGL(k_flow_blf<1>, dim3((w + BT_W - 1) / BT_W, (h + 7) / 8, bt.n), block, 0, s, out, in, img, ipitch, w, h, flow_pitch, blf_lut, bt.stride);
diff --git a/eppm_amd/csrc/k_prepare.hip b/eppm_amd/csrc/k_prepare.hip
--- a/eppm_amd/csrc/k_prepare.hip
+++ b/eppm_amd/csrc/k_prepare.hip
@@ -45,6 +45,57 @@
     vx /= sum; vy /= sum; vz /= sum; vw /= sum;
     const uint32_t r = (uint32_t)vx | ((uint32_t)vy << 8) | ((uint32_t)vz << 16) | ((uint32_t)vw << 24);
     out[y * pitch + x] = r;
+}
+
+__global__ __launch_bounds__(256) void k_gauss_rgba_direct(uint32_t* __restrict__ out0, uint32_t* __restrict__ raw0, uint32_t* __restrict__ out1,
+                                                           uint32_t* __restrict__ raw1, DirectFrames F, int in_pitch, int pitch, int h, int w,
+                                                           float sigma2, int radius, size_t pstride)
+{
+    const unsigned pair = blockIdx.z / 2, im = blockIdx.z % 2;
+    uint32_t* __restrict__ out = pair_ptr(im ? out1 : out0, pstride, pair);
+    uint32_t* __restrict__ raw = pair_ptr(im ? raw1 : raw0, pstride, pair);
+    const uint32_t* __restrict__ in = F.p[blockIdx.z];
+    __shared__ uint32_t tile[(GT_H + 2 * G_MAXR) * (GT_W + 2 * G_MAXR)];
+    __shared__ float wtab[(2 * G_MAXR + 1) * (2 * G_MAXR + 1)];
+    const int tw = GT_W + 2 * radius, th = GT_H + 2 * radius;
+    const int x0 = blockIdx.x * GT_W, y0 = blockIdx.y * GT_H;
+    const int tid = threadIdx.y * GT_W + threadIdx.x;
+    for (int t = tid; t < tw * th; t += 256) {
+        const int ty = t / tw, tx = t % tw;
+        const int cy = max(0, min(h - 1, y0 + ty - radius));
+        const int cx = max(0, min(w - 1, x0 + tx - radius));
+        tile[t] = in[(size_t)cy * in_pitch + cx];
+    }
+    const int d = 2 * radius + 1;
+    for (int t = tid; t < d * d; t += 256) {
+        const int dy = t / d - radius, dx = t % d - radius;
+        wtab[t] = fast_exp(-(float)(dy * dy + dx * dx) / sigma2);
+    }
+    __syncthreads();
+    const int x = x0 + threadIdx.x, y = y0 + threadIdx.y;
+    if (x >= w || y >= h) return;
+    raw[y * pitch + x] = tile[(threadIdx.y + radius) * tw + threadIdx.x + radius];
+    float vx = 0, vy = 0, vz = 0, vw = 0, sum = 0;
+    for (int dy = 0; dy < d; dy++)
+        for (int dx = 0; dx < d; dx++) {
+            const float weight = wtab[dy * d + dx];
+            const uint32_t p = tile[(threadIdx.y + dy) * tw + threadIdx.x + dx];
+            vx += (float)(p & 0xffu) * weight;
+            vy += (float)((p >> 8) & 0xffu) * weight;
+            vz += (float)((p >> 16) & 0xffu) * weight;
+            vw += (float)(p >> 24) * weight;
+            sum += weight;
+        }
+    vx /= sum; vy /= sum; vz /= sum; vw /= sum;
+    const uint32_t r = (uint32_t)vx | ((uint32_t)vy << 8) | ((uint32_t)vz << 16) | ((uint32_t)vw << 24);
+    out[y * pitch + x] = r;
+}
+bool prepare_direct_in(int npairs) { return EPPM_DIRECT_IO && npairs >= 1 && npairs <= kFlowOutsMax; }
+void launch_gauss_rgba2_direct(uint32_t* out0, uint32_t* raw0, uint32_t* out1, uint32_t* raw1, const DirectFrames& F, int in_pitch_px, int pitch_px,
+                               int h, int w, float sigma, int radius, hipStream_t s, Batch bt)
+{
+    dim3 grid((w + GT_W - 1) / GT_W, (h + GT_H - 1) / GT_H, 2 * bt.n), block(GT_W, GT_H);
+    hipLaunchKernelGGL(k_gauss_rgba_direct, grid, block, 0, s, out0, raw0, out1, raw1, F, in_pitch_px, pitch_px, h, w, sigma * sigma * 2, radius, bt.stride);
 }
 
 void launch_gauss_rgba(uint32_t* out, const uint32_t* in, int pitch_px, int h, int w, float sigma, int radius, hipStream_t s, Batch bt)
diff --git a/eppm_amd/csrc/launchers_ref_abi.cpp b/eppm_amd/csrc/launchers_ref_abi.cpp
--- a/eppm_amd/csrc/launchers_ref_abi.cpp
+++ b/eppm_amd/csrc/launchers_ref_abi.cpp
@@ -466,7 +466,13 @@
     PlanesH P;
     P.pk1 = a; P.pk2 = b; P.w = w; P.h = h; P.pitch = w;
     if (d_probe) HIPCHK(hipMemsetAsync(d_probe, 0xff, n * npairs * 73 * 4, g_stream));
-    launch_c2f_refine(P, (float*)f, ds->lut_pm, g_prm.patch_r, nullptr, g_stream, Batch{npairs, stride}, opt_no_split() != 0, pre, (unsigned*)st, d_probe);
+    void* rw = nullptr;
+    if (c2f_refine_wants_rest_weight(w, h, g_prm.patch_r, npairs, opt_no_split() != 0, false, d_probe ? 1 : pre, opt_c2f_restw())) {
+        CHK(get_scratch(ds, stride * npairs, &rw, 1));
+        launch_c2f_rest_weight(P, (float*)rw, ds->lut_pm, g_prm.patch_r, g_stream, Batch{npairs, stride});
+    }
+    launch_c2f_refine(P, (float*)f, ds->lut_pm, g_prm.patch_r, nullptr, g_stream, Batch{npairs, stride}, opt_no_split() != 0, pre, (unsigned*)st, d_probe,
+                      (const float*)rw);
     for (int p = 0; p < npairs; p++) CHK(copy_d2d(d_flow + p * n * 2, (char*)f + p * stride, n * 8));
     if (stat) { HIPCHK(hipMemcpyAsync(stat, st, 32, hipMemcpyDeviceToHost, g_stream)); HIPCHK(hipStreamSynchronize(g_stream)); }
     return finish();
@@ -487,6 +493,27 @@
 {
     if (!d_probe || g_prm.patch_r != 9) return set_err(EPPM_ERR_ARG, "eppm_test_c2f_refine_probe: bad argument (patch radius 9 only)");
     return c2f_refine_batch(d_flow, d_img1, d_img2, d_census1, d_census2, w, h, npairs, 1, nullptr, d_probe);
+}
+extern "C" int eppm_test_c2f_rest_weight(float* d_restw, const uint32_t* d_img1, const uint8_t* d_census1, int w, int h, int npairs)
+{
+#ifdef EPPM_TOL
+    (void)d_restw; (void)d_img1; (void)d_census1; (void)w; (void)h; (void)npairs;
+    return set_err(EPPM_ERR_ARG, "the tolerance library's window refine has no two-phase form");
+#else
+    if (!d_restw || !d_img1 || !d_census1 || w < 1 || h < 1 || npairs < 1 || g_prm.patch_r != 9)
+        return set_err(EPPM_ERR_ARG, "eppm_test_c2f_rest_weight: bad argument (patch radius 9 only)");
+    LAUNCHER_BEGIN_INT;
+    const size_t n = (size_t)w * h, stride = n * 16;
+    void *a = nullptr, *rw = nullptr;
+    CHK(get_scratch(ds, stride * npairs, &a, 2));
+    CHK(get_scratch(ds, stride * npairs, &rw, 1));
+    for (int p = 0; p < npairs; p++) launch_pack((char*)a + p * stride, w, d_img1 + p * n, w, d_census1 + p * n, w, w, h, g_stream);
+    PlanesH P;
+    P.pk1 = a; P.pk2 = a; P.w = w; P.h = h; P.pitch = w;
+    launch_c2f_rest_weight(P, (float*)rw, ds->lut_pm, 9, g_stream, Batch{npairs, stride});
+    for (int p = 0; p < npairs; p++) CHK(copy_d2d(d_restw + p * n, (char*)rw + p * stride, n * 4));
+    return finish();
+#endif
 }
 #endif
 
diff --git a/eppm_amd/stages.py b/eppm_amd/stages.py
--- a/eppm_amd/stages.py
+++ b/eppm_amd/stages.py
@@ -324,6 +324,16 @@
     return [out[k * h:(k + 1) * h] for k in range(n)], p[..., :36].reshape(n, h, w, 4, 9), p[..., 36:72].reshape(n, h, w, 4, 9), p[..., 72]
 
 
+def c2f_rest_weight(imgs, censuses):
+    n = len(imgs)
+    h, w = imgs[0].shape
+    i1, c1 = Dev(np.concatenate([np.ascontiguousarray(x) for x in imgs])), Dev(np.concatenate([np.ascontiguousarray(x) for x in censuses]))
+    rw = Dev(shape=(n * h, w), dtype=np.float32)
+    check(lib().eppm_test_c2f_rest_weight(rw.ptr, i1.ptr, c1.ptr, w, h, n), "eppm_test_c2f_rest_weight")
+    out = rw.get()
+    return [out[k * h:(k + 1) * h] for k in range(n)]
+
+
 def probe_c2f_pretest(patch_r=9):
     out, fl = _c2f_pretest_knobs(patch_r)
     return bool(out[0]), out[1], out[2], out[3], fl[0], fl[1], fl[2]
```

After: 255.9 Mflow-vectors/s, median of 6. About the same (+0.2%).
